# jklebes/MetropolisEngine

Measured on AMD Instinct MI355X. Metric: MC steps/sec (chains x sweeps) at 2^20 chains, 16 params, higher is better.
Workload: dtype f64

## Files before the change

### metropolisengine_amd/csrc/me_api.hip

```cpp
#include <algorithm>
#include <cmath>
#include <cstdlib>
#include <cstring>
#include <dlfcn.h>
#include <mutex>
#include <string>
#include <atomic>
#include <chrono>
#include <vector>

#include "me_comm.h"
#include "me_internal.h"

namespace me {

static std::vector<const KernelSet *> &registry() {
  static std::vector<const KernelSet *> sets;
  return sets;
}
static std::mutex &registry_mutex() {
  static std::mutex m;
  return m;
}
void register_kernel_set(const KernelSet *set) {
// ... 42 lines not shown
static bool host_factor(std::vector<double> &m, int nr, int nc) {
  auto tri = [](int i, int j) { return i * (i + 1) / 2 + j; };
  const int pr = nr * (nr + 1) / 2;
  auto cre = [pr](int i, int j) { return pr + i * i + 2 * j; };
  auto cim = [pr](int i, int j) { return pr + i * i + 2 * j + 1; };
  auto cdg = [pr](int i) { return pr + i * i + 2 * i; };
  for (int j = 0; j < nr; ++j) {
    double s = m[tri(j, j)];
    for (int k = 0; k < j; ++k) s -= m[tri(j, k)] * m[tri(j, k)];
    if (!(s > 0)) return false;
    const double dg = std::sqrt(s);
    m[tri(j, j)] = dg;
    for (int i = j + 1; i < nr; ++i) {
      double t = m[tri(i, j)];
      for (int k = 0; k < j; ++k) t -= m[tri(i, k)] * m[tri(j, k)];
      m[tri(i, j)] = t / dg;
    }
  }
  for (int j = 0; j < nc; ++j) {
    double s = m[cdg(j)];
    for (int k = 0; k < j; ++k) s -= m[cre(j, k)] * m[cre(j, k)] + m[cim(j, k)] * m[cim(j, k)];
    if (!(s > 0)) return false;
    const double dg = std::sqrt(s);
    m[cdg(j)] = dg;
    for (int i = j + 1; i < nc; ++i) {
      double tr = m[cre(i, j)], ti = m[cim(i, j)];
      for (int k = 0; k < j; ++k) {
        const double ar = m[cre(i, k)], ai = m[cim(i, k)], br = m[cre(j, k)], bi = m[cim(j, k)];
        tr -= ar * br + ai * bi;
        ti -= ai * br - ar * bi;
      }
      m[cre(i, j)] = tr / dg;
      m[cim(i, j)] = ti / dg;
    }
  }
  return true;
}

static bool initial_shape_is_identity(const me_config *c) {
  if (c->covariance_real)
    for (int i = 0; i < c->n_real; ++i)
      for (int j = 0; j <= i; ++j)
        if (c->covariance_real[i * c->n_real + j] != (i == j ? 1.0 : 0.0)) return false;
  if (c->covariance_complex)
    for (int i = 0; i < c->n_complex; ++i)
      for (int j = 0; j <= i; ++j) {
        const double re = c->covariance_complex[2 * (i * c->n_complex + j)], im = c->covariance_complex[2 * (i * c->n_complex + j) + 1];
        if (re != (i == j ? 1.0 : 0.0) || (i != j && im != 0.0)) return false;
      }
  return true;
}

}

using namespace me;

struct me_engine {
  int device = 0;
  hipStream_t stream = nullptr;
  bool own_stream = false;
  const KernelSet *ks = nullptr;
  int dtype = ME_F32;
  size_t esize = 4;
  long long n = 0;
  int nr = 0, nc = 0, d = 0, p = 0, nobs = 0;
  unsigned long long chain_offset = 0, seed = 0;
  double temp = 0, target_acceptance = 0.3, alpha = 0, ratio = 0, reject_bound = 0;
  int m = 0, energy_kind = 0, reject_kind = 0, cov_mode = 0;
  bool stale_total = false;
  hipEvent_t time_start = nullptr, time_stop = nullptr;
  std::vector<double> shared_host;
  int cov_kind = CK_IDENTITY;
  int grid_blocks = 0;
  int n_terms = 1;
  std::vector<double> coef;
  unsigned long long step_index = 0, measure_count = 1;
  unsigned long long fused_cycles = 0;
  void *x = nullptr, *energy = nullptr, *width = nullptr, *mean = nullptr, *cov = nullptr, *obs_mean = nullptr;
  void *factor = nullptr, *shared_factor = nullptr, *shared_full = nullptr, *shared_image = nullptr, *energy_image = nullptr, *coef_dev = nullptr,
       *row_dev = nullptr;
  unsigned long long *accept_slots = nullptr, *accept_total = nullptr;
  long long n_slots = 0;
  unsigned long long proposed = 0;
  bool x_tiled = false;
  int width_rows = 1;
  bool widths_synced = true;
  unsigned int *status = nullptr;
  double *pool_dev = nullptr, *pool_partials = nullptr, *pool_host = nullptr;
  unsigned long long *host_scratch = nullptr;
  hipStream_t copy_stream = nullptr;
  hipEvent_t pool_reduced = nullptr, pool_copied = nullptr;
  bool pool_pending = false;
  const RcclApi *rccl = nullptr;
  ncclComm_t comm = nullptr;
  int comm_rank = 0, comm_world = 1;
  double *trace_dev = nullptr;
  long long trace_chains = 0, trace_stride = 1, trace_rows = 0, trace_capacity = 0;
  std::string err;
};

namespace {

int fail(me_engine *e, int code, const std::string &msg) {
  if (e) e->err = msg;
  else g_create_error = msg;
  return code;
}

#define ME_HIP(e, call)                                                                                      \
  do {                                                                                                       \
    hipError_t err__ = (call);                                                                               \
    if (err__ != hipSuccess)                                                                                 \
      return fail((e), ME_ERR_HIP, std::string(#call) + ": " + hipGetErrorString(err__));                    \
  } while (0)

void to_device_type(const double *src, size_t count, int dtype, std::vector<unsigned char> &out) {
  out.resize(count * (dtype == ME_F32 ? 4 : 8));
  if (dtype == ME_F32) {
    float *o = reinterpret_cast<float *>(out.data());
    for (size_t i = 0; i < count; ++i) o[i] = (float)src[i];
  } else {
    std::memcpy(out.data(), src, count * 8);
  }
}

int broadcast(me_engine *e, void *dst, const std::vector<double> &row, bool tiled = false) {
  std::vector<unsigned char> bytes;
  to_device_type(row.data(), row.size(), e->dtype, bytes);
  ME_HIP(e, hipMemcpyAsync(e->row_dev, bytes.data(), bytes.size(), hipMemcpyHostToDevice, e->stream));
  if (tiled) ME_HIP(e, launch_broadcast_tiled(dst, e->row_dev, (int)row.size(), e->n, e->dtype, e->stream));
  else ME_HIP(e, launch_broadcast_rows(dst, e->row_dev, (int)row.size(), e->n, e->dtype, e->stream));
  ME_HIP(e, hipStreamSynchronize(e->stream));
  return ME_OK;
}

int check_status(me_engine *e);
int copy_tiled(me_engine *e, void *field_ptr, int entries, int64_t chain_begin, int64_t n_chains, double *dst, const double *src) {
  const int64_t tile0 = chain_begin >> 6, tile1 = (chain_begin + n_chains - 1) >> 6;
  const size_t tile_values = (size_t)entries * 64, n_values = (size_t)(tile1 - tile0 + 1) * tile_values;
  unsigned char *dev = (unsigned char *)field_ptr + (size_t)tile0 * tile_values * e->esize;
  std::vector<unsigned char> tmp(n_values * e->esize);
  const bool whole = (chain_begin & 63) == 0 && (((chain_begin + n_chains) & 63) == 0 || chain_begin + n_chains == e->n);
  if (dst || !whole) {
    ME_HIP(e, hipMemcpyAsync(tmp.data(), dev, tmp.size(), hipMemcpyDeviceToHost, e->stream));
    ME_HIP(e, hipStreamSynchronize(e->stream));
  }
  auto at = [&](int64_t c, int k) { return (size_t)((c >> 6) - tile0) * tile_values + (size_t)k * 64 + (size_t)(c & 63); };
  if (e->dtype == ME_F32) {
    float *t = reinterpret_cast<float *>(tmp.data());
    for (int64_t i = 0; i < n_chains; ++i)
      for (int k = 0; k < entries; ++k) {
        if (dst) dst[i * entries + k] = (double)t[at(chain_begin + i, k)];
        else t[at(chain_begin + i, k)] = (float)src[i * entries + k];
      }
  } else {
    double *t = reinterpret_cast<double *>(tmp.data());
    for (int64_t i = 0; i < n_chains; ++i)
      for (int k = 0; k < entries; ++k) {
        if (dst) dst[i * entries + k] = t[at(chain_begin + i, k)];
        else t[at(chain_begin + i, k)] = src[i * entries + k];
      }
  }
  if (src) {
    ME_HIP(e, hipMemcpyAsync(dev, tmp.data(), tmp.size(), hipMemcpyHostToDevice, e->stream));
    ME_HIP(e, hipStreamSynchronize(e->stream));
  }
  return dst ? check_status(e) : ME_OK;
}

int field_info(me_engine *e, int field, void **ptr, int *comps) {
  switch (field) {
    case ME_FIELD_PARAMS: *ptr = e->x; *comps = e->d; return ME_OK;
    case ME_FIELD_ENERGY: *ptr = e->energy; *comps = e->n_terms; return ME_OK;
    case ME_FIELD_WIDTH: *ptr = e->width; *comps = e->width_rows; return ME_OK;
    case ME_FIELD_MEAN: *ptr = e->mean; *comps = e->d; return ME_OK;
    case ME_FIELD_OBS_MEAN: *ptr = e->obs_mean; *comps = e->nobs; return ME_OK;
    case ME_FIELD_COV:
      if (!e->cov)
        return fail(e, ME_ERR_UNSUPPORTED, "this engine keeps no per-chain covariance: for large parameter spaces it is "
                                           "kept on request only (me_config.flags: ME_FLAG_TRACK_COVARIANCE), and not "
                                           "at all where the field would pass 4 GiB");
      *ptr = e->cov; *comps = e->p; return ME_OK;
    case ME_FIELD_ENERGY_TOTAL:
      if (!e->stale_total)
        return fail(e, ME_ERR_UNSUPPORTED, "this engine keeps one coherent energy ledger (sum ME_FIELD_ENERGY); a separate "
                                           "energy_total exists with ME_FLAG_REFERENCE_ENERGY_LEDGERS only");
      *ptr = (unsigned char *)e->energy + (size_t)e->n_terms * (size_t)e->n * e->esize; *comps = 1; return ME_OK;
    case ME_FIELD_FACTOR:
      if (!e->factor) return fail(e, ME_ERR_UNSUPPORTED, "this engine keeps no per-chain proposal factors (dimensions "
                                                         "without per-chain kernels, or a field beyond 4 GiB)");
      *ptr = e->factor; *comps = e->p; return ME_OK;
    default: return fail(e, ME_ERR_INVALID, "unknown field id");
  }
}

int report_status(me_engine *e, unsigned int bits) {
  if (!bits) return ME_OK;
  ME_HIP(e, hipMemsetAsync(e->status, 0, sizeof(unsigned int), e->stream));
  std::string msg = "numeric failure in at least one chain:";
  if (bits & ST_NONFINITE_ENERGY) msg += " non-finite energy;";
  if (bits & ST_BAD_PIVOT) msg += " non-positive Cholesky pivot (proposal covariance not positive definite);";
  if (bits & ST_BAD_WIDTH) msg += " sampling width <= 0;";
  return fail(e, ME_ERR_NUMERIC, msg);
}
int check_status(me_engine *e) {
  ME_HIP(e, hipMemcpyAsync(&e->host_scratch[0], e->status, sizeof(unsigned int), hipMemcpyDeviceToHost, e->stream));
  ME_HIP(e, hipStreamSynchronize(e->stream));
  return report_status(e, (unsigned int)e->host_scratch[0]);
}

int upload_shared_factor(me_engine *e, const double *packed) {
  std::vector<unsigned char> bytes;
  to_device_type(packed, (size_t)e->p, e->dtype, bytes);
  ME_HIP(e, hipMemcpy(e->shared_factor, bytes.data(), bytes.size(), hipMemcpyHostToDevice));
  if (e->shared_full) {
    std::vector<double> full((size_t)e->nr * e->nr, 0.0);
    for (int i = 0; i < e->nr; ++i)
      for (int j = 0; j <= i; ++j) full[(size_t)i * e->nr + j] = packed[i * (i + 1) / 2 + j];
    to_device_type(full.data(), full.size(), e->dtype, bytes);
    ME_HIP(e, hipMemcpy(e->shared_full, bytes.data(), bytes.size(), hipMemcpyHostToDevice));
    if (e->shared_image) ME_HIP(e, e->ks->prepare_matrix(e->shared_full, e->shared_image, e->stream));
  }
  return ME_OK;
}

void fill_step_launch(me_engine *e, StepLaunch &l, int n_sweeps) {
  l.n_real = e->nr;
  l.n_complex = e->nc;
  l.x = e->x;
  l.energy = e->energy;
// ... 129 lines not shown
      const bool dense = c->energy_kind == ME_ENERGY_DENSE_QUAD, pooled = c->cov_mode == ME_COV_POOLED || starts_shared;
      const bool per_chain = c->cov_mode == ME_COV_REFERENCE || (c->flags & ME_FLAG_TRACK_COVARIANCE) != 0;
      if ((dense || pooled || per_chain) && per_block * (pooled ? 2 : 1) > 150 * 1024)
        return fail(nullptr, ME_ERR_UNSUPPORTED,
                    "a dense quadratic form, a shared proposal factor or per-chain shapes beyond " + std::to_string(kMaxRegisterDof) +
                        " degrees of freedom are staged in LDS: this many parameters do not fit (float64: about 290, 145 with "
                        "a shared factor or an initial covariance that ME_COV_FIXED keeps; float32 twice that)");
    }
    if (c->flags & ME_FLAG_REFERENCE_ENERGY_LEDGERS)
      return fail(nullptr, ME_ERR_UNSUPPORTED, "ME_FLAG_REFERENCE_ENERGY_LEDGERS is not available beyond " +
                                                   std::to_string(kMaxRegisterDof) + " real degrees of freedom");
    if (c->reject_kind == ME_REJECT_USER) return fail(nullptr, ME_ERR_UNSUPPORTED, "no user plugins at these dimensions");
  }
  if ((c->flags & ME_FLAG_REFERENCE_ENERGY_LEDGERS) && (c->n_real == 0 || c->n_complex == 0))
    return fail(nullptr, ME_ERR_INVALID,
                "ME_FLAG_REFERENCE_ENERGY_LEDGERS applies to mixed engines (real and complex parameters): only their "
                "step_all keeps a separate energy_total (metropolis_engine.py:241-259)");
  if (c->cov_mode == ME_COV_REFERENCE && !ks->per_chain_cov)
    return fail(nullptr, ME_ERR_UNSUPPORTED,
                "per-chain adaptive covariance is not compiled for these dimensions; use ME_COV_FIXED or ME_COV_POOLED");

  bool keep_per_chain = ks->per_chain_cov && (!ks->streams_packed || c->cov_mode == ME_COV_REFERENCE);
  {
    const long long esz = c->dtype == ME_F32 ? 4 : 8;
    const long long limit = 1ll << 32;
    if (keep_per_chain && !ks->streams_packed && (long long)packed_total(c->n_real, c->n_complex) * ((c->n_chains + 63) / 64 * 64) * esz >= limit) {
      if (c->cov_mode == ME_COV_REFERENCE)
        return fail(nullptr, ME_ERR_UNSUPPORTED,
                    "the per-chain covariance field would exceed 4 GiB on this engine; shard the chains over more "
                    "engines or use ME_COV_FIXED / ME_COV_POOLED");
      keep_per_chain = false;
    }
    const long long rows = std::max<long long>(c->n_real + 2 * c->n_complex, 2 * c->n_real + c->n_complex);
    if (rows * ((c->n_chains + 63) / 64 * 64) * esz >= limit)
      return fail(nullptr, ME_ERR_UNSUPPORTED,
                  "a per-chain field would exceed 4 GiB on this engine; shard the chains over more engines");
  }
  int n_dev = 0;
  if (hipGetDeviceCount(&n_dev) != hipSuccess || n_dev <= 0)
    return fail(nullptr, ME_ERR_HIP, "no HIP device available (this library has no CPU fallback)");
  if (c->device_id < 0 || c->device_id >= n_dev) return fail(nullptr, ME_ERR_INVALID, "device_id out of range");

  me_engine *e = new me_engine;
  e->device = c->device_id;
  e->ks = ks;
  e->n_terms = ks->energy_terms(c->energy_kind);
  e->dtype = c->dtype;
  e->esize = c->dtype == ME_F32 ? 4 : 8;
  e->n = c->n_chains;
  e->nr = c->n_real;
  e->nc = c->n_complex;
  e->d = e->nr + 2 * e->nc;
  e->p = packed_total(e->nr, e->nc);
  e->nobs = n_observables(e->nr, e->nc);
  e->chain_offset = c->chain_offset;
  e->seed = c->seed;
  e->temp = c->temp;
  e->target_acceptance = c->target_acceptance;
  e->energy_kind = c->energy_kind;
  e->reject_kind = c->reject_kind;
  e->reject_bound = c->reject_bound;
  e->cov_mode = c->cov_mode;
  e->coef.assign(c->energy_coeffs, c->energy_coeffs + c->n_energy_coeffs);
  e->alpha = -norm_ppf(c->target_acceptance / 2.0);
  e->m = e->nr + e->nc;
  e->ratio = (1.0 - 1.0 / e->m) * std::sqrt(2.0 * M_PI) * std::exp(e->alpha * e->alpha / 2.0) / 2.0 * e->alpha +
             1.0 / (e->m * c->target_acceptance * (1.0 - c->target_acceptance));
  if (const char *g = std::getenv("ME_GRID_BLOCKS")) e->grid_blocks = std::atoi(g);

#define ME_CREATE_HIP(call)                                                                  \
  do {                                                                                       \
    hipError_t err__ = (call);                                                               \
    if (err__ != hipSuccess) {                                                               \
      g_create_error = std::string(#call) + ": " + hipGetErrorString(err__);                 \
      release(e);                                                                            \
      return ME_ERR_HIP;                                                                     \
    }                                                                                        \
  } while (0)

  ME_CREATE_HIP(hipSetDevice(e->device));
  ME_CREATE_HIP(hipStreamCreateWithFlags(&e->stream, hipStreamNonBlocking));
  e->own_stream = true;
  const size_t n = (size_t)e->n, es = e->esize;
  e->x_tiled = ks->tiled_state;
  ME_CREATE_HIP(hipMalloc(&e->x, (e->x_tiled ? (n + 63) / 64 * 64 : n) * e->d * es));
  e->stale_total = (c->flags & ME_FLAG_REFERENCE_ENERGY_LEDGERS) != 0;
  ME_CREATE_HIP(hipMalloc(&e->energy, n * (e->n_terms + (e->stale_total ? 1 : 0)) * es));
  e->width_rows = (e->nr > 0 && e->nc > 0) ? 3 : 1;
  ME_CREATE_HIP(hipMalloc(&e->width, n * e->width_rows * es));
  ME_CREATE_HIP(hipMalloc(&e->mean, n * e->d * es));
  ME_CREATE_HIP(hipMalloc(&e->obs_mean, n * e->nobs * es));
  if (keep_per_chain || ((!ks->per_chain_cov || ks->streams_packed) && ks->tracks_cov && (c->flags & ME_FLAG_TRACK_COVARIANCE)))
    ME_CREATE_HIP(hipMalloc(&e->cov, (n + 63) / 64 * 64 * e->p * es));
  if (keep_per_chain) ME_CREATE_HIP(hipMalloc(&e->factor, (n + 63) / 64 * 64 * e->p * es));
  ME_CREATE_HIP(hipMalloc(&e->shared_factor, (size_t)e->p * es));
  if (e->nc == 0) ME_CREATE_HIP(hipMalloc(&e->shared_full, (size_t)e->nr * e->nr * es));
  if (e->shared_full && ks->prepare_matrix) ME_CREATE_HIP(hipMalloc(&e->shared_image, ks->matrix_image_bytes));
  ME_CREATE_HIP(hipMalloc(&e->row_dev, (size_t)std::max(std::max(e->d, e->p), e->nobs) * es));
  e->n_slots = (e->n + 31) / 32 + 8;
  ME_CREATE_HIP(hipMalloc((void **)&e->accept_slots, (size_t)e->n_slots * sizeof(unsigned long long)));
  ME_CREATE_HIP(hipMalloc((void **)&e->accept_total, sizeof(unsigned long long)));
  ME_CREATE_HIP(hipMalloc((void **)&e->status, sizeof(unsigned int)));
  ME_CREATE_HIP(hipMalloc((void **)&e->pool_dev, sizeof(double) * (size_t)moments_size(e->nr, e->nc)));
  ME_CREATE_HIP(hipHostMalloc((void **)&e->host_scratch, 64, hipHostMallocDefault));
  e->host_scratch[0] = e->host_scratch[1] = 0;
  ME_CREATE_HIP(hipHostMalloc((void **)&e->pool_host, sizeof(double) * (size_t)moments_size(e->nr, e->nc), hipHostMallocDefault));
  if (pool_reduce_supported(e->nr, e->nc, e->dtype))
    ME_CREATE_HIP(hipMalloc((void **)&e->pool_partials,
                            sizeof(double) * (size_t)pool_reduce_blocks(e->n, e->nr, e->nc) *
                                (size_t)(1 + e->d + e->nr + e->nc + e->d * (e->d + 1) / 2)));
  ME_CREATE_HIP(hipMemsetAsync(e->accept_slots, 0, (size_t)e->n_slots * sizeof(unsigned long long), e->stream));
  ME_CREATE_HIP(hipMemsetAsync(e->status, 0, sizeof(unsigned int), e->stream));
  if (ks->n_real < 0 && e->energy_kind == ME_ENERGY_DIAG_QUAD) {
    if ((int)e->coef.size() != e->nr + e->nc) {
      g_create_error = "wrong number of energy coefficients for this energy kind";
      release(e);
      return ME_ERR_INVALID;
    }
    std::vector<double> expanded(e->coef.begin(), e->coef.begin() + e->nr);
    expanded.insert(expanded.end(), e->coef.begin() + e->nr, e->coef.end());
    expanded.insert(expanded.end(), e->coef.begin() + e->nr, e->coef.end());
    std::vector<unsigned char> bytes;
    to_device_type(expanded.data(), expanded.size(), e->dtype, bytes);
    ME_CREATE_HIP(hipMalloc(&e->coef_dev, bytes.size()));
    ME_CREATE_HIP(hipMemcpy(e->coef_dev, bytes.data(), bytes.size(), hipMemcpyHostToDevice));
  }
  if (ks->n_real < 0 && e->energy_kind == ME_ENERGY_DENSE_QUAD) {
    if ((int)e->coef.size() != e->d * e->d) {
      g_create_error = "wrong number of energy coefficients for this energy kind";
      release(e);
      return ME_ERR_INVALID;
    }
    std::vector<double> folded;
    folded.reserve((size_t)e->d * (e->d + 1) / 2);
    for (int i = 0; i < e->d; ++i)
      for (int j = 0; j <= i; ++j)
        folded.push_back(i == j ? e->coef[(size_t)i * e->d + i] : e->coef[(size_t)i * e->d + j] + e->coef[(size_t)j * e->d + i]);
    std::vector<unsigned char> bytes;
    to_device_type(folded.data(), folded.size(), e->dtype, bytes);
    ME_CREATE_HIP(hipMalloc(&e->coef_dev, bytes.size()));
    ME_CREATE_HIP(hipMemcpy(e->coef_dev, bytes.data(), bytes.size(), hipMemcpyHostToDevice));
  } else
  if (e->energy_kind == ME_ENERGY_DENSE_QUAD || (is_user_kind(e->energy_kind) && !e->coef.empty())) {
    std::vector<unsigned char> bytes;
    to_device_type(e->coef.data(), e->coef.size(), e->dtype, bytes);
    ME_CREATE_HIP(hipMalloc(&e->coef_dev, bytes.size()));
    ME_CREATE_HIP(hipMemcpy(e->coef_dev, bytes.data(), bytes.size(), hipMemcpyHostToDevice));
    if (e->energy_kind == ME_ENERGY_DENSE_QUAD && ks->prepare_matrix) {
      ME_CREATE_HIP(hipMalloc(&e->energy_image, ks->matrix_image_bytes));
      ME_CREATE_HIP(ks->prepare_matrix(e->coef_dev, e->energy_image, e->stream));
    }
  }
#undef ME_CREATE_HIP

  std::vector<double> init(c->initial_params, c->initial_params + e->d);
  std::vector<double> obs(e->nobs);
  for (int i = 0; i < e->nr; ++i) {
    obs[i] = std::fabs(init[i]);
    obs[e->nr + e->nc + i] = init[i] * init[i];
  }
  for (int j = 0; j < e->nc; ++j) obs[e->nr + j] = std::hypot(init[e->nr + j], init[e->nr + e->nc + j]);
  const int pr = packed_real(e->nr);
  std::vector<double> c0(e->p, 0.0);
  bool identity = true;
  for (int i = 0; i < e->nr; ++i)
    for (int j = 0; j <= i; ++j) {
      const double v = c->covariance_real ? c->covariance_real[i * e->nr + j] : (i == j ? 1.0 : 0.0);
      c0[i * (i + 1) / 2 + j] = v;
      identity = identity && v == (i == j ? 1.0 : 0.0);
    }
  for (int i = 0; i < e->nc; ++i) {
    for (int j = 0; j < i; ++j) {
      const double re = c->covariance_complex ? c->covariance_complex[2 * (i * e->nc + j)] : 0.0;
      const double im = c->covariance_complex ? c->covariance_complex[2 * (i * e->nc + j) + 1] : 0.0;
      c0[pr + i * i + 2 * j] = re;
      c0[pr + i * i + 2 * j + 1] = im;
      identity = identity && re == 0.0 && im == 0.0;
    }
    const double dg = c->covariance_complex ? c->covariance_complex[2 * (i * e->nc + i)] : 1.0;
    c0[pr + i * i + 2 * i] = dg;
    identity = identity && dg == 1.0;
  }
  std::vector<double> f0 = c0;
  for (int i = 0; i < e->nc; ++i)
    for (int j = 0; j < i; ++j) f0[pr + i * i + 2 * j + 1] = -f0[pr + i * i + 2 * j + 1];
  if (!host_factor(f0, e->nr, e->nc)) {
    release(e);
    return fail(nullptr, ME_ERR_INVALID, "initial covariance matrix is not positive definite (metropolis_engine.py:270)");
  }
  int rc = ME_OK;
  std::vector<double> width_row((size_t)e->width_rows, c->sampling_width);
  if ((rc = broadcast(e, e->x, init, e->x_tiled)) || (rc = broadcast(e, e->mean, init)) || (rc = broadcast(e, e->obs_mean, obs)) ||
      (rc = broadcast(e, e->width, width_row)) || (e->cov && (rc = broadcast(e, e->cov, c0, true))) ||
      (e->factor && (rc = broadcast(e, e->factor, f0, true)))) {
    g_create_error = e->err;
    release(e);
    return rc;
  }
  if (upload_shared_factor(e, f0.data()) != ME_OK) {
    g_create_error = e->err;
    release(e);
    return ME_ERR_HIP;
  }
  e->cov_kind = identity ? CK_IDENTITY : (ks->n_real < 0 && e->factor) ? CK_PER_CHAIN : CK_SHARED;

  rc = me_recompute_energy(e);
  if (rc == ME_OK) {
    hipError_t herr = hipStreamSynchronize(e->stream);
    if (herr != hipSuccess) rc = fail(e, ME_ERR_HIP, std::string("initial energy evaluation: ") + hipGetErrorString(herr));
  }
  if (rc != ME_OK) {
    g_create_error = e->err;
    release(e);
    return rc;
  }
  *out = e;
  return ME_OK;
}

int me_set_reject_condition(me_engine *e, int32_t reject_kind, double reject_bound) {
  if (!e) return ME_ERR_INVALID;
  if (reject_kind < ME_REJECT_NONE || reject_kind > ME_REJECT_USER) return fail(e, ME_ERR_INVALID, "unknown reject_kind");
  if (reject_kind == ME_REJECT_USER && e->energy_kind != ME_ENERGY_USER && e->energy_kind != ME_ENERGY_USER_INDIRECT)
    return fail(e, ME_ERR_INVALID, "ME_REJECT_USER needs a user-energy plugin (it supplies me_user_reject)");
  if (reject_kind == ME_REJECT_USER && !e->ks->has_user_reject)
    return fail(e, ME_ERR_UNSUPPORTED,
                "ME_REJECT_USER: this user-energy plugin defines no me_user_reject (#define ME_USER_HAS_REJECT in its source)");
  if (reject_kind == ME_REJECT_ABS_REAL0_GE && e->nr == 0)
    return fail(e, ME_ERR_INVALID, "ME_REJECT_ABS_REAL0_GE needs a real parameter");
  e->reject_kind = reject_kind;
  e->reject_bound = reject_bound;
  return ME_OK;
}

int me_set_energy(me_engine *e, int32_t energy_kind, const double *coeffs, int32_t n_coeffs, const char *user_name) {
  if (!e) return ME_ERR_INVALID;
  if (n_coeffs < 0 || (n_coeffs > 0 && !coeffs)) return fail(e, ME_ERR_INVALID, "energy coefficients missing");
  if (e->ks->n_real < 0) return fail(e, ME_ERR_UNSUPPORTED, "me_set_energy: not available on the runtime-dimension kernel set");
  if (energy_kind == ME_ENERGY_DENSE_QUAD)
    return fail(e, ME_ERR_UNSUPPORTED, "me_set_energy: the dense quadratic form keeps device images of its matrix; create a new engine");
  const KernelSet *ks = find_kernel_set(e->dtype, e->nr, e->nc, energy_kind, user_name);
  if (!ks || ks->n_real < 0)
    return fail(e, ME_ERR_UNSUPPORTED, is_user_kind(energy_kind)
                    ? std::string("no user-energy plugin named '") + (user_name ? user_name : "") + "' is loaded for these dimensions"
                    : "energy kind " + std::to_string(energy_kind) + " is not compiled for these dimensions");
  if (ks->tiled_state != e->ks->tiled_state || ks->per_chain_cov != e->ks->per_chain_cov || ks->streams_packed != e->ks->streams_packed ||
      ks->tracks_cov != e->ks->tracks_cov)
    return fail(e, ME_ERR_UNSUPPORTED, "me_set_energy: the plugin was built with other per-chain covariance options than this engine's kernel set");
  if (e->reject_kind == ME_REJECT_USER && !ks->has_user_reject)
    return fail(e, ME_ERR_UNSUPPORTED, "me_set_energy: the engine's wall is the plugin's me_user_reject, which the new energy does not define");
  const int n_terms = ks->energy_terms(energy_kind);
  ME_HIP(e, hipSetDevice(e->device));
  ME_HIP(e, hipStreamSynchronize(e->stream));
  if (n_terms != e->n_terms) {
    void *ledger = nullptr;
    ME_HIP(e, hipMalloc(&ledger, (size_t)e->n * (size_t)(n_terms + (e->stale_total ? 1 : 0)) * e->esize));
    (void)hipFree(e->energy);
    e->energy = ledger;
    e->n_terms = n_terms;
    if (e->trace_chains > 0) {
      if (e->trace_dev) (void)hipFree(e->trace_dev);
      e->trace_dev = nullptr;
      e->trace_rows = e->trace_capacity = 0;
    }
  }
  e->coef.assign(coeffs, coeffs + n_coeffs);
  if (e->coef_dev) {
    (void)hipFree(e->coef_dev);
    e->coef_dev = nullptr;
  }
  if (is_user_kind(energy_kind) && !e->coef.empty()) {
    std::vector<unsigned char> bytes;
    to_device_type(e->coef.data(), e->coef.size(), e->dtype, bytes);
    ME_HIP(e, hipMalloc(&e->coef_dev, bytes.size()));
    ME_HIP(e, hipMemcpy(e->coef_dev, bytes.data(), bytes.size(), hipMemcpyHostToDevice));
  }
  e->ks = ks;
  e->energy_kind = energy_kind;
  const int rc = me_recompute_energy(e);
  if (rc != ME_OK) return rc;
  ME_HIP(e, hipStreamSynchronize(e->stream));
  return check_status(e);
}

int me_load_plugin(const char *path) {
  if (!path) return fail(nullptr, ME_ERR_INVALID, "null plugin path");
  void *handle = dlopen(path, RTLD_NOW | RTLD_GLOBAL);
  if (!handle) return fail(nullptr, ME_ERR_INVALID, std::string("dlopen failed: ") + dlerror());
  return ME_OK;
}

int me_destroy(me_engine *e) {
  if (!e) return ME_ERR_INVALID;
  (void)hipSetDevice(e->device);
  if (e->stream) (void)hipStreamSynchronize(e->stream);
  if (e->copy_stream) (void)hipStreamSynchronize(e->copy_stream);
  release(e);
  return ME_OK;
}

int me_recompute_energy(me_engine *e) {
  if (!e) return ME_ERR_INVALID;
  ME_HIP(e, hipSetDevice(e->device));
  EnergyLaunch l;
  l.n_real = e->nr;
  l.n_complex = e->nc;
  l.total_row = e->stale_total ? e->n_terms : -1;
  l.x = e->x;
  l.energy = e->energy;
  l.coef_device = e->coef_dev;
  l.coef_host = e->coef.data();
  l.n_coef = (int)e->coef.size();
  l.status = e->status;
  l.n = e->n;
  l.energy_kind = e->energy_kind;
  l.grid_blocks = e->grid_blocks;
  hipError_t err = e->ks->init_energy(l, e->stream);
  if (err == hipErrorInvalidValue) return fail(e, ME_ERR_INVALID, "wrong number of energy coefficients for this energy kind");
  ME_HIP(e, err);
  return ME_OK;
}

static int split_widths(me_engine *e) {
  if (e->width_rows != 3 || !e->widths_synced) return ME_OK;
  const size_t row = (size_t)e->n * e->esize;
  for (int r = 1; r <= 2; ++r)
    ME_HIP(e, hipMemcpyAsync((unsigned char *)e->width + r * row, e->width, row, hipMemcpyDeviceToDevice, e->stream));
  e->widths_synced = false;
  return ME_OK;
// ... 45 lines not shown

int me_step(me_engine *e, int32_t n_sweeps) { return me_step_kind(e, ME_STEP_ALL, n_sweeps); }

int me_step_kind(me_engine *e, int32_t kind, int32_t n_sweeps) {
  if (!e) return ME_ERR_INVALID;
  if (n_sweeps <= 0) return fail(e, ME_ERR_INVALID, "n_sweeps must be positive");
  ME_HIP(e, hipSetDevice(e->device));
  return launch_step_kind(e, kind, n_sweeps, nullptr, nullptr);
}

int me_step_injected(me_engine *e, int32_t kind, int32_t n_sweeps, const double *normals, const double *uniforms) {
  if (!e || !normals || !uniforms) return ME_ERR_INVALID;
  if (n_sweeps <= 0) return fail(e, ME_ERR_INVALID, "n_sweeps must be positive");
  if (e->dtype != ME_F64) return fail(e, ME_ERR_UNSUPPORTED, "injected-stream replay is compiled for float64 engines only");
  ME_HIP(e, hipSetDevice(e->device));
  const bool magphase = kind == ME_STEP_COMPLEX_MAGNITUDE_PHASE;
  const size_t n = (size_t)e->n, k = (size_t)n_sweeps;
  const size_t nz = magphase ? (size_t)e->nc : (size_t)e->d, nu = magphase ? (size_t)e->nc + 2 : 1;
  std::vector<double> zn(k * nz * n), un(k * nu * n);
  for (size_t s = 0; s < k; ++s)
    for (size_t c = 0; c < n; ++c) {
      for (size_t j = 0; j < nz; ++j) zn[(s * nz + j) * n + c] = normals[(s * n + c) * nz + j];
      for (size_t j = 0; j < nu; ++j) un[(s * nu + j) * n + c] = uniforms[(s * n + c) * nu + j];
    }
  double *zd = nullptr, *ud = nullptr;
  ME_HIP(e, hipMalloc((void **)&zd, zn.size() * sizeof(double)));
  hipError_t herr = hipMalloc((void **)&ud, un.size() * sizeof(double));
  if (herr != hipSuccess) {
    (void)hipFree(zd);
    return fail(e, ME_ERR_HIP, "hipMalloc of the injected uniforms failed");
  }
  int rc = ME_OK;
  if (hipMemcpy(zd, zn.data(), zn.size() * sizeof(double), hipMemcpyHostToDevice) != hipSuccess ||
      hipMemcpy(ud, un.data(), un.size() * sizeof(double), hipMemcpyHostToDevice) != hipSuccess) {
    rc = fail(e, ME_ERR_HIP, "upload of the injected streams failed");
  } else {
    rc = launch_step_kind(e, kind, n_sweeps, zd, ud);
    if (rc == ME_OK && hipStreamSynchronize(e->stream) != hipSuccess) rc = fail(e, ME_ERR_HIP, "injected step failed");
  }
  (void)hipFree(zd);
  (void)hipFree(ud);
  return rc;
}

namespace {
void fill_measure_launch(me_engine *e, MeasureLaunch &l, unsigned long long count) {
  l.n_real = e->nr;
  l.n_complex = e->nc;
  l.x = e->x;
  l.width = e->width;
  l.mean = e->mean;
  l.cov = e->cov;
  l.obs_mean = e->obs_mean;
  l.factor = e->factor;
  l.status = e->status;
  l.n = e->n;
  l.measure_count = count;
  l.update_cov = (count > 50 && e->cov) ? 1 : 0;
  l.split_widths = (e->width_rows == 3 && !e->widths_synced) ? 1 : 0;
  l.write_factor = (l.update_cov && e->cov_mode == ME_COV_REFERENCE) ? 1 : 0;
  l.grid_blocks = e->grid_blocks;
}

int commit_measure(me_engine *e, const MeasureLaunch &l) {
  e->measure_count = l.measure_count;
  if (l.write_factor) e->cov_kind = CK_PER_CHAIN;
  if (e->trace_chains > 0) {
    const long long cols = e->d + e->n_terms + e->width_rows;
    if (e->trace_rows == e->trace_capacity) {
      const long long cap = e->trace_capacity ? 2 * e->trace_capacity : 1024;
      double *bigger = nullptr;
      ME_HIP(e, hipMalloc((void **)&bigger, sizeof(double) * (size_t)(cap * cols * e->trace_chains)));
      if (e->trace_dev) {
        ME_HIP(e, hipMemcpyAsync(bigger, e->trace_dev, sizeof(double) * (size_t)(e->trace_rows * cols * e->trace_chains),
                                 hipMemcpyDeviceToDevice, e->stream));
        ME_HIP(e, hipStreamSynchronize(e->stream));
        (void)hipFree(e->trace_dev);
      }
      e->trace_dev = bigger;
      e->trace_capacity = cap;
    }
    const int rows_valid = (e->width_rows == 3 && e->widths_synced) ? 1 : e->width_rows;
    ME_HIP(e, launch_trace(e->x, e->energy, e->width, e->n, e->d, e->n_terms, rows_valid, e->dtype, e->trace_chains, e->trace_stride,
                           e->trace_dev + e->trace_rows * cols * e->trace_chains, e->stream, e->x_tiled));
    if (rows_valid != e->width_rows) {
      double *row = e->trace_dev + e->trace_rows * cols * e->trace_chains + (size_t)(e->d + e->n_terms) * e->trace_chains;
      for (int r = 1; r < 3; ++r)
        ME_HIP(e, hipMemcpyAsync(row + (size_t)r * e->trace_chains, row, sizeof(double) * (size_t)e->trace_chains,
                                 hipMemcpyDeviceToDevice, e->stream));
    }
    e->trace_rows += 1;
  }
  return ME_OK;
}
}

int me_measure(me_engine *e) {
  if (!e) return ME_ERR_INVALID;
  ME_HIP(e, hipSetDevice(e->device));
  MeasureLaunch l;
  fill_measure_launch(e, l, e->measure_count + 1);
  ME_HIP(e, e->ks->measure(l, e->stream));
  return commit_measure(e, l);
}

int me_cycle(me_engine *e, int32_t n_sweeps) {
  if (!e) return ME_ERR_INVALID;
  if (n_sweeps <= 0) return fail(e, ME_ERR_INVALID, "n_sweeps must be positive");
  ME_HIP(e, hipSetDevice(e->device));
  if (e->ks->cycle) {
    StepLaunch sl;
    fill_step_launch(e, sl, n_sweeps);
    MeasureLaunch ml;
    fill_measure_launch(e, ml, e->measure_count + 1);
    ml.split_widths = 0;
    const hipError_t err = e->ks->cycle(sl, ml, e->stream);
    if (err == hipSuccess) {
      e->widths_synced = true;
      e->step_index += (unsigned long long)n_sweeps;
      e->proposed += (unsigned long long)e->n * (unsigned long long)n_sweeps;
      e->fused_cycles += 1;
      return commit_measure(e, ml);
    }
    if (err != hipErrorNotSupported) ME_HIP(e, err);
    (void)hipGetLastError();
  }
  const int rc = me_step(e, n_sweeps);
  return rc != ME_OK ? rc : me_measure(e);
}

int me_cycle_stats(me_engine *e, uint64_t *fused_cycles) {
  if (!e || !fused_cycles) return ME_ERR_INVALID;
  *fused_cycles = e->fused_cycles;
  return ME_OK;
}

int me_trace_enable(me_engine *e, int64_t n_traced, int64_t stride) {
  if (!e) return ME_ERR_INVALID;
  if (n_traced < 0 || stride < 1 || (n_traced > 0 && (n_traced - 1) * stride >= e->n))
    return fail(e, ME_ERR_INVALID, "traced chains out of range");
  ME_HIP(e, hipSetDevice(e->device));
  ME_HIP(e, hipStreamSynchronize(e->stream));
  if (e->trace_dev) (void)hipFree(e->trace_dev);
  e->trace_dev = nullptr;
  e->trace_chains = n_traced;
  e->trace_stride = stride;
  e->trace_rows = e->trace_capacity = 0;
  return ME_OK;
}

int me_trace_shape(me_engine *e, int64_t *rows, int64_t *cols, int64_t *n_traced) {
  if (!e) return ME_ERR_INVALID;
  if (rows) *rows = e->trace_rows;
  if (cols) *cols = e->d + e->n_terms + e->width_rows;
  if (n_traced) *n_traced = e->trace_chains;
  return ME_OK;
}

int me_trace_get(me_engine *e, double *dst, int64_t n_doubles) {
  if (!e || !dst) return ME_ERR_INVALID;
  const long long want = e->trace_rows * (e->d + e->n_terms + e->width_rows) * e->trace_chains;
  if (n_doubles != want) return fail(e, ME_ERR_INVALID, "wrong trace buffer length");
  if (want == 0) return ME_OK;
  ME_HIP(e, hipSetDevice(e->device));
  ME_HIP(e, hipStreamSynchronize(e->stream));
  ME_HIP(e, hipMemcpy(dst, e->trace_dev, sizeof(double) * (size_t)want, hipMemcpyDeviceToHost));
  return ME_OK;
}

int me_field_components(me_engine *e, int32_t field, int32_t *n_components) {
  if (!e || !n_components) return ME_ERR_INVALID;
  void *ptr;
  int comps;
  int rc = field_info(e, field, &ptr, &comps);
  if (rc == ME_OK) *n_components = comps;
  return rc;
}

int me_energy_terms(me_engine *e, int32_t *n_terms) {
  if (!e || !n_terms) return ME_ERR_INVALID;
  *n_terms = e->n_terms;
  return ME_OK;
}

int me_get(me_engine *e, int32_t field, int64_t chain_begin, int64_t n_chains, double *dst) {
  if (!e || !dst) return ME_ERR_INVALID;
  if (chain_begin < 0 || n_chains < 0 || chain_begin + n_chains > e->n) return fail(e, ME_ERR_INVALID, "chain range out of bounds");
  ME_HIP(e, hipSetDevice(e->device));
  void *ptr;
  int comps;
  int rc = field_info(e, field, &ptr, &comps);
  if (rc != ME_OK) return rc;
  if (n_chains == 0) return ME_OK;
  if (field == ME_FIELD_COV || field == ME_FIELD_FACTOR || (field == ME_FIELD_PARAMS && e->x_tiled))
    return copy_tiled(e, ptr, comps, chain_begin, n_chains, dst, nullptr);
  std::vector<unsigned char> tmp((size_t)comps * n_chains * e->esize);
  for (int r = 0; r < comps; ++r)
    ME_HIP(e, hipMemcpyAsync(tmp.data() + (size_t)r * n_chains * e->esize,
                             (const unsigned char *)ptr + ((size_t)r * e->n + chain_begin) * e->esize,
                             (size_t)n_chains * e->esize, hipMemcpyDeviceToHost, e->stream));
  ME_HIP(e, hipStreamSynchronize(e->stream));
  if (e->dtype == ME_F32) {
    const float *t = reinterpret_cast<const float *>(tmp.data());
    for (int r = 0; r < comps; ++r)
      for (int64_t c = 0; c < n_chains; ++c) dst[c * comps + r] = (double)t[(size_t)r * n_chains + c];
  } else {
    const double *t = reinterpret_cast<const double *>(tmp.data());
    for (int r = 0; r < comps; ++r)
      for (int64_t c = 0; c < n_chains; ++c) dst[c * comps + r] = t[(size_t)r * n_chains + c];
  }
  if (field == ME_FIELD_WIDTH && e->width_rows == 3 && e->widths_synced)
    for (int64_t c = 0; c < n_chains; ++c) dst[c * 3 + 1] = dst[c * 3 + 2] = dst[c * 3];
  return check_status(e);
}

int me_set(me_engine *e, int32_t field, int64_t chain_begin, int64_t n_chains, const double *src) {
  if (!e || !src) return ME_ERR_INVALID;
  if (chain_begin < 0 || n_chains < 0 || chain_begin + n_chains > e->n) return fail(e, ME_ERR_INVALID, "chain range out of bounds");
  ME_HIP(e, hipSetDevice(e->device));
  void *ptr;
  int comps;
  int rc = field_info(e, field, &ptr, &comps);
  if (rc != ME_OK) return rc;
  if (field == ME_FIELD_WIDTH && e->width_rows == 3 && (chain_begin != 0 || n_chains != e->n))
    return fail(e, ME_ERR_INVALID, "widths of a mixed engine must be set for all chains at once");
  if (n_chains == 0) return ME_OK;
  if (field == ME_FIELD_COV || field == ME_FIELD_FACTOR || (field == ME_FIELD_PARAMS && e->x_tiled)) {
    rc = copy_tiled(e, ptr, comps, chain_begin, n_chains, nullptr, src);
    if (rc != ME_OK) return rc;
    if (field == ME_FIELD_FACTOR) e->cov_kind = CK_PER_CHAIN;
    return ME_OK;
  }
  std::vector<unsigned char> tmp((size_t)comps * n_chains * e->esize);
  if (e->dtype == ME_F32) {
    float *t = reinterpret_cast<float *>(tmp.data());
    for (int r = 0; r < comps; ++r)
      for (int64_t c = 0; c < n_chains; ++c) t[(size_t)r * n_chains + c] = (float)src[c * comps + r];
  } else {
    double *t = reinterpret_cast<double *>(tmp.data());
    for (int r = 0; r < comps; ++r)
      for (int64_t c = 0; c < n_chains; ++c) t[(size_t)r * n_chains + c] = src[c * comps + r];
  }
  for (int r = 0; r < comps; ++r)
    ME_HIP(e, hipMemcpyAsync((unsigned char *)ptr + ((size_t)r * e->n + chain_begin) * e->esize,
                             tmp.data() + (size_t)r * n_chains * e->esize, (size_t)n_chains * e->esize,
                             hipMemcpyHostToDevice, e->stream));
  ME_HIP(e, hipStreamSynchronize(e->stream));
  if (field == ME_FIELD_FACTOR) e->cov_kind = CK_PER_CHAIN;
  if (field == ME_FIELD_WIDTH && e->width_rows == 3) e->widths_synced = false;
  return ME_OK;
}

int me_constants(me_engine *e, double *alpha, int32_t *m, double *ratio) {
  if (!e) return ME_ERR_INVALID;
  if (alpha) *alpha = e->alpha;
  if (m) *m = e->m;
  if (ratio) *ratio = e->ratio;
  return ME_OK;
}

int me_counters(me_engine *e, uint64_t *step_index, uint64_t *measure_step_counter) {
  if (!e) return ME_ERR_INVALID;
  if (step_index) *step_index = e->step_index;
  if (measure_step_counter) *measure_step_counter = e->measure_count;
  return ME_OK;
}

int me_set_counters(me_engine *e, uint64_t step_index, uint64_t measure_step_counter) {
  if (!e) return ME_ERR_INVALID;
  if (measure_step_counter < 1) return fail(e, ME_ERR_INVALID, "measure_step_counter starts at 1");
  e->step_index = step_index;
  e->measure_count = measure_step_counter;
  return ME_OK;
}

int me_accept_stats(me_engine *e, uint64_t *accepted, uint64_t *proposed) {
  if (!e) return ME_ERR_INVALID;
  ME_HIP(e, hipSetDevice(e->device));
  ME_HIP(e, launch_sum_slots(e->accept_slots, e->n_slots, e->accept_total, e->stream));
  ME_HIP(e, hipMemcpyAsync(&e->host_scratch[1], e->accept_total, sizeof(unsigned long long), hipMemcpyDeviceToHost, e->stream));
  ME_HIP(e, hipMemcpyAsync(&e->host_scratch[0], e->status, sizeof(unsigned int), hipMemcpyDeviceToHost, e->stream));
  ME_HIP(e, hipStreamSynchronize(e->stream));
  if (accepted) *accepted = e->host_scratch[1];
  if (proposed) *proposed = e->proposed;
  return report_status(e, (unsigned int)e->host_scratch[0]);
}

int me_set_accept_stats(me_engine *e, uint64_t accepted, uint64_t proposed) {
  if (!e) return ME_ERR_INVALID;
  if (accepted > proposed) return fail(e, ME_ERR_INVALID, "accepted exceeds proposed");
  ME_HIP(e, hipSetDevice(e->device));
  const unsigned long long total = accepted;
  ME_HIP(e, hipMemsetAsync(e->accept_slots, 0, (size_t)e->n_slots * sizeof(unsigned long long), e->stream));
  ME_HIP(e, hipMemcpyAsync(e->accept_slots, &total, sizeof(total), hipMemcpyHostToDevice, e->stream));
  ME_HIP(e, hipStreamSynchronize(e->stream));
  e->proposed = proposed;
  return ME_OK;
}

int me_pooled_moments_size(me_engine *e, int64_t *n_doubles) {
  if (!e || !n_doubles) return ME_ERR_INVALID;
  *n_doubles = moments_size(e->nr, e->nc);
  return ME_OK;
}

namespace {
int enqueue_pooled_moments(me_engine *e, void *device_out, int64_t n_doubles) {
  if (n_doubles != moments_size(e->nr, e->nc)) return fail(e, ME_ERR_INVALID, "wrong pooled-moment buffer length");
  if (e->pool_pending) return fail(e, ME_ERR_STATE, "a pooled-moment reduction is in flight (me_pooled_moments_end first)");
  if (!e->pool_partials) return fail(e, ME_ERR_UNSUPPORTED, "pooled moments: dimension too large for the reduction kernel");
  ME_HIP(e, hipSetDevice(e->device));
  hipError_t err = launch_pool_reduce(e->x, e->n, e->nr, e->nc, e->dtype, e->accept_slots, e->n_slots,
                                      (double)e->proposed, e->pool_partials, (double *)device_out, e->stream,
                                      e->ks->pool_stage1, e->x_tiled);
  if (err == hipErrorInvalidValue) return fail(e, ME_ERR_UNSUPPORTED, "pooled moments: dimension too large for the reduction kernel");
  ME_HIP(e, err);
  return ME_OK;
}
}

static hipError_t wait_polling(hipEvent_t ev) {
  const auto t0 = std::chrono::steady_clock::now();
  for (;;) {
    const hipError_t rc = hipEventQuery(ev);
    if (rc != hipErrorNotReady) return rc;
    if (std::chrono::steady_clock::now() - t0 > std::chrono::milliseconds(2)) return hipEventSynchronize(ev);
  }
}
static hipError_t wait_polling(hipStream_t stream) {
  const auto t0 = std::chrono::steady_clock::now();
  for (;;) {
    const hipError_t rc = hipStreamQuery(stream);
    if (rc != hipErrorNotReady) return rc;
    if (std::chrono::steady_clock::now() - t0 > std::chrono::milliseconds(2)) return hipStreamSynchronize(stream);
  }
}

int me_pooled_moments_device(me_engine *e, void *device_out, int64_t n_doubles) {
  if (!e || !device_out) return ME_ERR_INVALID;
  int rc = enqueue_pooled_moments(e, device_out, n_doubles);
  if (rc != ME_OK) return rc;
  ME_HIP(e, wait_polling(e->stream));
  return ME_OK;
}

int me_pooled_moments(me_engine *e, double *host_out, int64_t n_doubles) {
  if (!e || !host_out) return ME_ERR_INVALID;
  int rc = enqueue_pooled_moments(e, e->pool_dev, n_doubles);
  if (rc != ME_OK) return rc;
  ME_HIP(e, hipMemcpyAsync(e->pool_host, e->pool_dev, sizeof(double) * (size_t)n_doubles, hipMemcpyDeviceToHost, e->stream));
  ME_HIP(e, wait_polling(e->stream));
  std::memcpy(host_out, e->pool_host, sizeof(double) * (size_t)n_doubles);
  return ME_OK;
}

namespace {
int begin_pooled(me_engine *e, bool allreduce) {
  if (e->pool_pending) return fail(e, ME_ERR_STATE, "a pooled-moment reduction is already in flight: call me_pooled_moments_end first");
  if (allreduce && !e->comm)
    return fail(e, ME_ERR_STATE, "this engine has no communicator: call me_comm_init_rank first (single-GPU engines use me_pooled_moments)");
  ME_HIP(e, hipSetDevice(e->device));
  if (!e->copy_stream) {
    ME_HIP(e, hipStreamCreateWithFlags(&e->copy_stream, hipStreamNonBlocking));
    ME_HIP(e, hipEventCreateWithFlags(&e->pool_reduced, hipEventDisableTiming));
    ME_HIP(e, hipEventCreateWithFlags(&e->pool_copied, hipEventDisableTiming));
  }
  const int64_t n_doubles = moments_size(e->nr, e->nc);
  int rc = enqueue_pooled_moments(e, e->pool_dev, n_doubles);
  if (rc != ME_OK) return rc;
  ME_HIP(e, hipEventRecord(e->pool_reduced, e->stream));
  ME_HIP(e, hipStreamWaitEvent(e->copy_stream, e->pool_reduced, 0));
  if (allreduce) {
    const ncclResult_t nrc = e->rccl->all_reduce(e->pool_dev, e->pool_dev, (size_t)n_doubles, ncclDouble, ncclSum, e->comm, e->copy_stream);
    if (nrc != ncclSuccess) return fail(e, ME_ERR_HIP, std::string("ncclAllReduce: ") + e->rccl->error_string(nrc));
  }
  ME_HIP(e, hipMemcpyAsync(e->pool_host, e->pool_dev, sizeof(double) * (size_t)n_doubles, hipMemcpyDeviceToHost, e->copy_stream));
  ME_HIP(e, hipEventRecord(e->pool_copied, e->copy_stream));
  e->pool_pending = true;
  return ME_OK;
}
}

int me_pooled_moments_begin(me_engine *e) {
  if (!e) return ME_ERR_INVALID;
  return begin_pooled(e, false);
}

int me_pooled_moments_allreduce_begin(me_engine *e) {
  if (!e) return ME_ERR_INVALID;
  return begin_pooled(e, true);
}

int me_pooled_moments_allreduce(me_engine *e, double *host_out, int64_t n_doubles) {
  if (!e || !host_out) return ME_ERR_INVALID;
  if (n_doubles != moments_size(e->nr, e->nc)) return fail(e, ME_ERR_INVALID, "wrong pooled-moment buffer length");
  const int rc = begin_pooled(e, true);
  return rc != ME_OK ? rc : me_pooled_moments_end(e, host_out, n_doubles);
// ... 193 lines not shown
```

### metropolisengine_amd/csrc/me_device.h

```cpp
#pragma once

#include <type_traits>
#include <utility>

#include <hip/hip_runtime.h>
#include <stdint.h>

#include "me_internal.h"
#include "me_math64.h"

namespace me {

struct U4 {
  uint32_t x, y, z, w;
};

__device__ __forceinline__ uint32_t xor3(uint32_t a, uint32_t b, uint32_t c) {
  return __builtin_amdgcn_bitop3_b32(a, b, c, 0x96);
}
__device__ __forceinline__ U4 philox4x32_10(U4 c, uint32_t k0, uint32_t k1) {
#pragma unroll
  for (int r = 0; r < 10; ++r) {
    const uint64_t p0 = (uint64_t)0xD2511F53u * c.x;
    const uint64_t p1 = (uint64_t)0xCD9E8D57u * c.z;
// ... 111 lines not shown
                                            (unsigned int)row * row_bytes, ME_NT_AUX);
    } else {
      using v2 = decltype(__builtin_amdgcn_raw_buffer_load_b64(rsrc, 0u, 0u, 0));
      __builtin_amdgcn_raw_buffer_store_b64(__builtin_bit_cast(v2, value), rsrc, chain_off,
                                            (unsigned int)row * row_bytes, ME_NT_AUX);
    }
  }
  __device__ __forceinline__ void store(int row, unsigned int chain_off, R value) const {
    if constexpr (sizeof(R) == 4) {
      __builtin_amdgcn_raw_buffer_store_b32(__builtin_bit_cast(unsigned int, value), rsrc, chain_off,
                                            (unsigned int)row * row_bytes, 0);
    } else {
      using v2 = decltype(__builtin_amdgcn_raw_buffer_load_b64(rsrc, 0u, 0u, 0));
      __builtin_amdgcn_raw_buffer_store_b64(__builtin_bit_cast(v2, value), rsrc, chain_off,
                                            (unsigned int)row * row_bytes, 0);
    }
  }
};

template <typename R>
__device__ __forceinline__ unsigned int tiled_offset(long long c, int entries) {
  return (unsigned int)(((c >> 6) * (long long)entries * 64 + (c & 63)) * (long long)sizeof(R));
}
template <typename R>
struct TiledField {
  __amdgpu_buffer_rsrc_t rsrc;
  __device__ __forceinline__ TiledField(const R *base, long long n, int entries)
      : rsrc(__builtin_amdgcn_make_buffer_rsrc(const_cast<R *>(base), 0,
                                               (unsigned int)(((n + 63) >> 6) * (long long)entries * 64 * (long long)sizeof(R)),
                                               0x00020000)) {}
  static constexpr unsigned int kEntryBytes = 64u * (unsigned int)sizeof(R);
  template <int AUX>
  __device__ __forceinline__ R load_aux(int k, unsigned int tile_off) const {
    if constexpr (sizeof(R) == 4) {
      return __builtin_bit_cast(R, __builtin_amdgcn_raw_buffer_load_b32(rsrc, tile_off, (unsigned int)k * kEntryBytes, AUX));
    } else {
      const auto v = __builtin_amdgcn_raw_buffer_load_b64(rsrc, tile_off, (unsigned int)k * kEntryBytes, AUX);
      return __builtin_bit_cast(R, v);
    }
  }
  template <int AUX>
  __device__ __forceinline__ void store_aux(int k, unsigned int tile_off, R value) const {
    if constexpr (sizeof(R) == 4) {
      __builtin_amdgcn_raw_buffer_store_b32(__builtin_bit_cast(unsigned int, value), rsrc, tile_off, (unsigned int)k * kEntryBytes, AUX);
    } else {
      using v2 = decltype(__builtin_amdgcn_raw_buffer_load_b64(rsrc, 0u, 0u, 0));
      __builtin_amdgcn_raw_buffer_store_b64(__builtin_bit_cast(v2, value), rsrc, tile_off, (unsigned int)k * kEntryBytes, AUX);
    }
  }
  __device__ __forceinline__ R load(int k, unsigned int tile_off) const { return load_aux<0>(k, tile_off); }
  __device__ __forceinline__ R load_nt(int k, unsigned int tile_off) const { return load_aux<ME_NT_AUX>(k, tile_off); }
  __device__ __forceinline__ void store(int k, unsigned int tile_off, R value) const { store_aux<0>(k, tile_off, value); }
  __device__ __forceinline__ void store_nt(int k, unsigned int tile_off, R value) const { store_aux<ME_NT_AUX>(k, tile_off, value); }
};

template <bool NT, class F>
__device__ __forceinline__ auto packed_load(const F &f, int row, unsigned int chain_off) {
  if constexpr (NT) return f.load_nt(row, chain_off);
  else return f.load(row, chain_off);
}
template <bool NT, class F, typename R>
__device__ __forceinline__ void packed_store(const F &f, int row, unsigned int chain_off, R value) {
  if constexpr (NT) f.store_nt(row, chain_off, value);
  else f.store(row, chain_off, value);
}

template <typename R, bool NTS>
struct StateField : Field<R> {
  using Field<R>::Field;
  __device__ __forceinline__ R load(int row, unsigned int chain_off) const {
    if constexpr (NTS) return Field<R>::load_nt(row, chain_off);
    else return Field<R>::load(row, chain_off);
  }
  __device__ __forceinline__ void store(int row, unsigned int chain_off, R value) const {
    if constexpr (NTS) Field<R>::store_nt(row, chain_off, value);
    else Field<R>::store(row, chain_off, value);
  }
};

#ifndef ME_TILED_STATE_DOF
#define ME_TILED_STATE_DOF 16
#endif
constexpr int kTiledStateDof = ME_TILED_STATE_DOF;
template <typename R, int D, bool NTS = false>
struct XField {
  static constexpr bool kTiled = D >= kTiledStateDof;
  std::conditional_t<kTiled, TiledField<R>, StateField<R, NTS>> f;
  __device__ __forceinline__ XField(const R *base, long long n) : f(base, n, D) {}
  static __device__ __forceinline__ unsigned int offset(long long c) {
    if constexpr (kTiled) return tiled_offset<R>(c, D);
    else return (unsigned int)c * (unsigned int)sizeof(R);
  }
  __device__ __forceinline__ R load(int row, unsigned int off) const {
    if constexpr (kTiled && NTS) return f.load_nt(row, off);
    else return f.load(row, off);
  }
  __device__ __forceinline__ void store(int row, unsigned int off, R value) const {
    if constexpr (kTiled && NTS) f.store_nt(row, off, value);
    else f.store(row, off, value);
  }
};
template <typename R, int D>
__device__ __forceinline__ long long state_index(long long c, int row, long long n) {
  if constexpr (D >= kTiledStateDof) return ((c >> 6) * (long long)D + row) * 64 + (c & 63);
  else return (long long)row * n + c;
}

constexpr int kMaxPackedInRegisters = 160;
#ifndef ME_STREAM_F64_ENTRIES
#define ME_STREAM_F64_ENTRIES 96
#endif
constexpr int kStreamF64Entries = ME_STREAM_F64_ENTRIES;

template <typename R, int NR, int NC>
struct EnergyIso {
  static constexpr int D = NR + 2 * NC;
  R a;
  __device__ __forceinline__ R operator()(const R (&x)[D]) const {
    R s0 = 0, s1 = 0;
#pragma unroll
    for (int d = 0; d + 1 < D; d += 2) {
      s0 += x[d] * x[d];
      s1 += x[d + 1] * x[d + 1];
    }
    if constexpr (D % 2 == 1) s0 += x[D - 1] * x[D - 1];
    return a * (s0 + s1);
  }
};

template <typename R, int NR, int NC>
struct EnergyDiag {
  static constexpr int D = NR + 2 * NC;
  R w[D];
  __device__ __forceinline__ R operator()(const R (&x)[D]) const {
    R s0 = 0, s1 = 0;
#pragma unroll
    for (int d = 0; d + 1 < D; d += 2) {
      s0 += w[d] * x[d] * x[d];
      s1 += w[d + 1] * x[d + 1] * x[d + 1];
    }
    if constexpr (D % 2 == 1) s0 += w[D - 1] * x[D - 1] * x[D - 1];
    return s0 + s1;
  }
};

template <typename R, int NR, int NC>
struct EnergyDense {
  static constexpr int D = NR + 2 * NC;
  static constexpr int PT = D * (D + 1) / 2;
  const R *a;
  static __device__ __forceinline__ R *folded() {
    __shared__ R t[PT];
    return t;
  }
  __device__ __forceinline__ void prepare() const {
    R *t = folded();
    constexpr int kBatch = 8;
    for (int k0 = threadIdx.x; k0 < PT; k0 += kBatch * (int)blockDim.x) {
      R lo[kBatch], hi[kBatch];
#pragma unroll
      for (int u = 0; u < kBatch; ++u) {
        const int k = k0 + u * (int)blockDim.x;
        lo[u] = hi[u] = R(0);
        if (k < PT) {
          int i = (int)((__builtin_sqrtf((float)(8 * k + 1)) - 1.0f) * 0.5f);
          if ((i + 1) * (i + 2) / 2 <= k) ++i;
          if (i * (i + 1) / 2 > k) --i;
          const int j = k - i * (i + 1) / 2;
          lo[u] = a[i * D + j];
          if (i != j) hi[u] = a[j * D + i];
        }
      }
#pragma unroll
      for (int u = 0; u < kBatch; ++u) {
        const int k = k0 + u * (int)blockDim.x;
        if (k < PT) t[k] = lo[u] + hi[u];
      }
    }
    __syncthreads();
  }
  __device__ __forceinline__ R operator()(const R (&x)[D]) const {
    const R *t = folded();
    asm volatile("" ::: "memory");
    R e = 0;
#pragma unroll
    for (int i = 0; i < D; ++i) {
      R y = 0;
#pragma unroll
// ... 185 lines not shown
#pragma unroll
    for (int j = 0; j < D; ++j) g[j] = a.inj_normals[((long long)s * D + j) * a.n + c];
    u = a.inj_uniforms[(long long)s * a.n + c];
  } else {
    uint32_t words[4 * NBLK];
#pragma unroll
    for (int b = 0; b < NBLK; ++b) {
      U4 ctr;
      ctr.x = (uint32_t)gid;
      ctr.y = (uint32_t)(gid >> 32);
      ctr.z = (uint32_t)step;
      ctr.w = ((uint32_t)(step >> 32) << 16) | (uint32_t)b;
      const U4 o = philox4x32_10(ctr, a.seed_lo, a.seed_hi);
      words[4 * b + 0] = o.x;
      words[4 * b + 1] = o.y;
      words[4 * b + 2] = o.z;
      words[4 * b + 3] = o.w;
    }
#pragma unroll
    for (int q = 0; q < NW / 2; ++q) N_::normal_pair(words[2 * q], words[2 * q + 1], g[2 * q], g[2 * q + 1]);
    u = N_::unit(words[NW]);
  }

}

template <typename R, int NR, int NC, int CK, int GROUP, class Fac>
__device__ __forceinline__ void propose_registers(const R (&x)[NR + 2 * NC], const R (&g)[2 * ((NR + 2 * NC + 1) / 2)], R w_r, R w_c,
                                                  Fac &&fac, R (&xp)[NR + 2 * NC]) {
  constexpr int D = NR + 2 * NC;
  [[maybe_unused]] constexpr int PR = NR * (NR + 1) / 2;
  constexpr bool MOVE_REAL = NR > 0 && GROUP != GROUP_COMPLEX;
  constexpr bool MOVE_COMPLEX = NC > 0 && GROUP != GROUP_REAL;
#pragma unroll
  for (int d = 0; d < D; ++d) xp[d] = x[d];
  if constexpr (CK == CK_IDENTITY) {
    if constexpr (MOVE_REAL) {
#pragma unroll
      for (int i = 0; i < NR; ++i) xp[i] = x[i] + w_r * g[i];
    }
    if constexpr (MOVE_COMPLEX) {
#pragma unroll
      for (int j = 0; j < NC; ++j) {
        xp[NR + j] = x[NR + j] + w_c * (g[NR + j] * R(0.70710678118654752440));
        xp[NR + NC + j] = x[NR + NC + j] + w_c * (g[NR + NC + j] * R(0.70710678118654752440));
      }
    }
  } else {
    if constexpr (MOVE_REAL) {
#pragma unroll
      for (int i = 0; i < NR; ++i) {
        R acc = 0;
#pragma unroll
        for (int j = 0; j <= i; ++j) acc += fac(tri(i, j)) * g[j];
        xp[i] = x[i] + w_r * acc;
      }
    }
    if constexpr (MOVE_COMPLEX) {
#pragma unroll
      for (int i = 0; i < NC; ++i) {
        R are = 0, aim = 0;
#pragma unroll
        for (int j = 0; j < i; ++j) {
          const R lre = fac(cre(PR, i, j));
          const R lim = fac(cim(PR, i, j));
          const R wre = g[NR + j] * R(0.70710678118654752440), wim = g[NR + NC + j] * R(0.70710678118654752440);
          are += lre * wre - lim * wim;
          aim += lre * wim + lim * wre;
        }
        const R ld = fac(cdiag(PR, i));
        are += ld * (g[NR + i] * R(0.70710678118654752440));
        aim += ld * (g[NR + NC + i] * R(0.70710678118654752440));
        xp[NR + i] = x[NR + i] + w_c * are;
        xp[NR + NC + i] = x[NR + NC + i] + w_c * aim;
      }
    }
  }

}

template <typename R, int NR, int NC, class Energy, int CK, int GROUP, class Ledger>
__device__ __forceinline__ void decide_step(const StepArgs<R> &a, const Energy &en, bool stale_total, R u,
                                            const R (&g)[2 * ((NR + 2 * NC + 1) / 2)], R (&x)[NR + 2 * NC], const R (&xp)[NR + 2 * NC],
                                            Ledger &ledger, R &total_q5, R &w, R &w_r, R &w_c, unsigned int &wave_accepted,
                                            bool &bad_energy) {
  [[maybe_unused]] constexpr int D = NR + 2 * NC;
  constexpr bool MOVE_REAL = NR > 0 && GROUP != GROUP_COMPLEX;
  constexpr bool MOVE_COMPLEX = NC > 0 && GROUP != GROUP_REAL;
  using N_ = Num<R>;
  bool rejected = false;
  if (a.reject_kind == ME_REJECT_ABS_REAL0_GE) rejected = !(N_::abs_(xp[0]) < a.reject_bound);
  else if (a.reject_kind == ME_REJECT_USER) rejected = energy_reject(en, xp, 0);
  R terms_new[Ledger::T];
  const R e_new = ledger.propose(en, xp, terms_new);
  const R diff = e_new - (stale_total ? total_q5 : ledger.partial());
  bool accept = diff <= R(0);
  if (a.temp > R(0)) accept = accept || N_::uphill(u, diff, a.inv_temp, a.inv_temp_log2e);
  accept = accept && !rejected;
  bad_energy |= (!rejected && !N_::finite(e_new));
  if constexpr (CK == CK_IDENTITY) {
    const R wa_r = accept ? w_r : R(0), wa_c = accept ? w_c : R(0);
    if constexpr (MOVE_REAL) {
#pragma unroll
      for (int i = 0; i < NR; ++i) x[i] = x[i] + wa_r * g[i];
    }
    if constexpr (MOVE_COMPLEX) {
#pragma unroll
      for (int j = 0; j < NC; ++j) {
        x[NR + j] = x[NR + j] + wa_c * (g[NR + j] * R(0.70710678118654752440));
        x[NR + NC + j] = x[NR + NC + j] + wa_c * (g[NR + NC + j] * R(0.70710678118654752440));
      }
    }
  } else {
#pragma unroll
    for (int d = 0; d < D; ++d) x[d] = accept ? xp[d] : x[d];
  }
  if (stale_total) total_q5 = accept ? e_new : total_q5;
  else ledger.commit(accept, terms_new);
  w = N_::adapt(w, accept, a.ratio, a.p, a.damping, a.up, a.down);
  if constexpr (GROUP == GROUP_ALL) w_r = w_c = w;
  else if constexpr (GROUP == GROUP_REAL) w_r = w;
  else w_c = w;
  wave_accepted += (unsigned int)__popcll(__ballot(accept));
}

template <typename R, int NR, int NC, class Energy, int CK, bool INJECT, int GROUP, class Ledger, class Fac>
__device__ __forceinline__ void run_sweeps(const StepArgs<R> &a, const Energy &en, long long c, unsigned long long gid,
                                           bool stale_total, R (&x)[NR + 2 * NC], Ledger &ledger, R &total_q5, R &w, R &w_r,
                                           R &w_c, Fac &&fac, unsigned int &wave_accepted, bool &bad_energy) {
  constexpr int D = NR + 2 * NC;
  constexpr int NW = 2 * ((D + 1) / 2);
  for (int s = 0; s < a.n_sweeps; ++s) {
    R g[NW], u, xp[D];
    draw_step<R, NR, NC, INJECT>(a, c, gid, s, g, u);
    propose_registers<R, NR, NC, CK, GROUP>(x, g, w_r, w_c, fac, xp);
    decide_step<R, NR, NC, Energy, CK, GROUP>(a, en, stale_total, u, g, x, xp, ledger, total_q5, w, w_r, w_c, wave_accepted, bad_energy);
  }
}

#ifndef ME_STEP_WAVES_PER_EU
#define ME_STEP_WAVES_PER_EU 0
#endif
#if ME_STEP_WAVES_PER_EU > 0
#define ME_STEP_BOUNDS __launch_bounds__(kFusedStepThreads, ME_STEP_WAVES_PER_EU)
#else
#define ME_STEP_BOUNDS __launch_bounds__(kFusedStepThreads)
#endif

#ifndef ME_STEP_PRIO_SHIFT
#define ME_STEP_PRIO_SHIFT 8
#endif
__device__ __forceinline__ void stagger_priority() {
#if ME_STEP_PRIO_SHIFT >= 0
  switch ((blockIdx.x >> ME_STEP_PRIO_SHIFT) & 3u) {
    case 0: __builtin_amdgcn_s_setprio(3); break;
    case 1: __builtin_amdgcn_s_setprio(2); break;
    case 2: __builtin_amdgcn_s_setprio(1); break;
    default: break;
  }
#endif
}

template <typename R, int NR, int NC, class Energy, int CK, bool INJECT = false, int GROUP = GROUP_ALL, bool NTS = false>
__global__ void ME_STEP_BOUNDS k_step(StepArgs<R> a, Energy en) {
  constexpr int D = NR + 2 * NC;
  constexpr bool MIXED = NR > 0 && NC > 0;
  static_assert(GROUP == GROUP_ALL || MIXED, "group-wise kernels exist for mixed engines only");
  using N_ = Num<R>;

  stagger_priority();
  if constexpr (!INJECT) N_::prepare();
  energy_prepare(en, 0);
  unsigned int wave_accepted = 0;
  bool bad_energy = false, bad_width = false;
  const long long stride = (long long)gridDim.x * blockDim.x;
  using Ledger = EnergyLedger<R, Energy, GROUP>;
  const XField<R, D, NTS> fx(a.x, a.n);
  const StateField<R, NTS> fe(a.energy, a.n, Ledger::T + (MIXED ? 1 : 0)), fw(a.width, a.n, MIXED ? 3 : 1);
  const bool stale_total = MIXED && GROUP == GROUP_ALL && a.stale_total != 0;
  constexpr bool PER_CHAIN = CK == CK_PER_CHAIN || CK == CK_PER_CHAIN_NT;
  constexpr int PF = PER_CHAIN ? NR * (NR + 1) / 2 + NC * NC : 0;
  constexpr bool STREAM_FACTOR = PER_CHAIN && (PF > kMaxPackedInRegisters ||
                                               (!INJECT && sizeof(R) == 8 && NC == 0 && PF > kStreamF64Entries));
  const TiledField<R> ffac(a.factor, a.n, STREAM_FACTOR ? 0 : PF);
  for (long long c = (long long)blockIdx.x * blockDim.x + threadIdx.x; c < a.n; c += stride) {
    const unsigned int coff = (unsigned int)c * (unsigned int)sizeof(R);
    const unsigned int xoff = fx.offset(c);
    R x[D];
#pragma unroll
    for (int d = 0; d < D; ++d) x[d] = fx.load(d, xoff);
    Ledger ledger;
    R total_q5 = R(0);
    if (stale_total) total_q5 = fe.load(Ledger::T, coff);
    else ledger.load(fe, coff);
    R w = fw.load(MIXED ? GROUP : 0, coff);
    R w_r = w, w_c = w;
    if constexpr (MIXED && GROUP == GROUP_ALL) {
      if (a.split_widths) {
        w_r = fw.load(GROUP_REAL, coff);
        w_c = fw.load(GROUP_COMPLEX, coff);
      }
    }
    const unsigned long long gid = a.chain_offset + (unsigned long long)c;
    [[maybe_unused]] const unsigned int toff = tiled_offset<R>(c, PF);
    auto fac = [&](int k) -> R {
      if constexpr (CK == CK_PER_CHAIN_NT) return ffac.load_nt(k, toff);
      else if constexpr (CK == CK_PER_CHAIN) return ffac.load(k, toff);
      else return a.factor[k];
    };

    if constexpr (STREAM_FACTOR) {
      constexpr int NW = 2 * ((D + 1) / 2);
      for (int s = 0; s < a.n_sweeps; ++s) {
        static_assert(!INJECT, "the streamed-factor form has no replay hook");
        constexpr int NBLK = (NW + 1 + 3) / 4;
        const unsigned long long step = a.step_index + (unsigned long long)s;
        R g[NW];
        R u_accept;
        {
          uint32_t words[4 * NBLK];
#pragma unroll
          for (int b = 0; b < NBLK; ++b) {
            U4 ctr;
            ctr.x = (uint32_t)gid;
            ctr.y = (uint32_t)(gid >> 32);
            ctr.z = (uint32_t)step;
            ctr.w = ((uint32_t)(step >> 32) << 16) | (uint32_t)b;
            const U4 o = philox4x32_10(ctr, a.seed_lo, a.seed_hi);
            words[4 * b + 0] = o.x;
            words[4 * b + 1] = o.y;
            words[4 * b + 2] = o.z;
            words[4 * b + 3] = o.w;
          }
#pragma unroll
          for (int q = 0; q < NW / 2; ++q) N_::normal_pair(words[2 * q], words[2 * q + 1], g[2 * q], g[2 * q + 1]);
          u_accept = N_::unit(words[NW]);
        }
        R xp[D];
#pragma unroll
        for (int d = 0; d < D; ++d) xp[d] = x[d];
        asm volatile("" ::: "memory");
        constexpr int CH = (int)(ME_STREAM_CHUNK_BYTES / sizeof(R));
        const R *tile_base = a.factor + (c >> 6) * (long long)PF * 64;
        const unsigned long long tb = (unsigned long long)tile_base;
        const R *tile_uniform = (const R *)join_halves(__builtin_amdgcn_readfirstlane((int)(tb >> 32)),
                                                       __builtin_amdgcn_readfirstlane((int)(unsigned int)tb));
        const __amdgpu_buffer_rsrc_t tile = __builtin_amdgcn_make_buffer_rsrc(const_cast<R *>(tile_uniform), 0,
                                                                               (unsigned int)(PF * 64 * sizeof(R)), 0x00020000);
        const unsigned int lane_off = (unsigned int)(c & 63) * (unsigned int)sizeof(R);
        auto entry = [&](int k) -> R {
          constexpr int AUX = CK == CK_PER_CHAIN_NT ? ME_NT_AUX : 0;
          if constexpr (sizeof(R) == 4)
            return __builtin_bit_cast(R, __builtin_amdgcn_raw_buffer_load_b32(tile, lane_off, (unsigned int)k * 64u * 4u, AUX));
          else
            return __builtin_bit_cast(R, __builtin_amdgcn_raw_buffer_load_b64(tile, lane_off, (unsigned int)k * 64u * 8u, AUX));
        };
        R f[2][CH];
#pragma unroll
        for (int u = 0; u < CH; ++u)
          if (u < PF) f[0][u] = entry(u);
        auto use = [&](auto entry_index) -> R {
          constexpr int k = decltype(entry_index)::value;
          if constexpr (k % CH == 0) {
            __builtin_amdgcn_sched_barrier(0);
#pragma unroll
            for (int u = 0; u < CH; ++u)
              if (k + CH + u < PF) f[(k / CH + 1) & 1][u] = entry(k + CH + u);
            __builtin_amdgcn_sched_barrier(0);
          }
          return f[(k / CH) & 1][k % CH];
        };
        static_for<NR>([&](auto row_index) {
          constexpr int i = decltype(row_index)::value;
          R acc = 0;
          static_for<i + 1>([&](auto col_index) {
            constexpr int j = decltype(col_index)::value, k = tri(i, j);
            const R l = use(std::integral_constant<int, k>{});
            acc = j == 0 ? l * g[0] : acc + l * g[j];
          });
          if constexpr (GROUP != GROUP_COMPLEX) xp[i] = x[i] + w_r * acc;
        });
        static_for<NC>([&](auto row_index) {
          constexpr int i = decltype(row_index)::value;
          R are = 0, aim = 0;
          static_for<i>([&](auto col_index) {
            constexpr int j = decltype(col_index)::value;
            const R lre = use(std::integral_constant<int, cre(NR * (NR + 1) / 2, i, j)>{});
            const R lim = use(std::integral_constant<int, cim(NR * (NR + 1) / 2, i, j)>{});
            const R wre = g[NR + j] * R(0.70710678118654752440), wim = g[NR + NC + j] * R(0.70710678118654752440);
            are += lre * wre - lim * wim;
            aim += lre * wim + lim * wre;
          });
          const R ld = use(std::integral_constant<int, cdiag(NR * (NR + 1) / 2, i)>{});
          are += ld * (g[NR + i] * R(0.70710678118654752440));
          aim += ld * (g[NR + NC + i] * R(0.70710678118654752440));
          if constexpr (GROUP != GROUP_REAL) {
            xp[NR + i] = x[NR + i] + w_c * are;
            xp[NR + NC + i] = x[NR + NC + i] + w_c * aim;
          }
        });
        bool rejected = false;
        if (a.reject_kind == ME_REJECT_ABS_REAL0_GE) rejected = !(N_::abs_(xp[0]) < a.reject_bound);
        else if (a.reject_kind == ME_REJECT_USER) rejected = energy_reject(en, xp, 0);
        R terms_new[Ledger::T];
        const R e_new = ledger.propose(en, xp, terms_new);
        const R diff = e_new - (stale_total ? total_q5 : ledger.partial());
        bool accept = diff <= R(0);
        if (a.temp > R(0)) accept = accept || N_::uphill(u_accept, diff, a.inv_temp, a.inv_temp_log2e);
        accept = accept && !rejected;
        bad_energy |= (!rejected && !N_::finite(e_new));
#pragma unroll
        for (int d = 0; d < D; ++d) x[d] = accept ? xp[d] : x[d];
        if (stale_total) total_q5 = accept ? e_new : total_q5;
        else ledger.commit(accept, terms_new);
        w = N_::adapt(w, accept, a.ratio, a.p, a.damping, a.up, a.down);
        if constexpr (GROUP == GROUP_ALL) w_r = w_c = w;
        else if constexpr (GROUP == GROUP_REAL) w_r = w;
        else w_c = w;
        wave_accepted += (unsigned int)__popcll(__ballot(accept));
      }
    } else {
      run_sweeps<R, NR, NC, Energy, CK, INJECT, GROUP>(a, en, c, gid, stale_total, x, ledger, total_q5, w, w_r, w_c, fac, wave_accepted, bad_energy);
    }
    bad_width |= !(w > R(0));
#pragma unroll
    for (int d = 0; d < D; ++d) fx.store(d, xoff, x[d]);
    if (stale_total) fe.store(Ledger::T, coff, total_q5);
    else ledger.store(fe, coff);
    fw.store(MIXED ? GROUP : 0, coff, w);
  }
  if ((threadIdx.x & 63) == 0 && wave_accepted) {
    unsigned long long *slot = a.accept_slots + (size_t)blockIdx.x * (blockDim.x >> 6) + (threadIdx.x >> 6);
    *slot += (unsigned long long)wave_accepted;
  }
  const unsigned int bits = (bad_energy ? ST_NONFINITE_ENERGY : 0u) | (bad_width ? ST_BAD_WIDTH : 0u);
  if (bits) atomicOr(a.status, bits);
}

template <typename R, int NR, int NC, class Energy>
__global__ void __launch_bounds__(kStepThreads) k_init_energy(const R *xs, R *energy, long long n, unsigned int *status,
                                                                Energy en, int total_row) {
  constexpr int D = NR + 2 * NC;
  energy_prepare(en, 0);
  const long long stride = (long long)gridDim.x * kStepThreads;
  for (long long c = (long long)blockIdx.x * kStepThreads + threadIdx.x; c < n; c += stride) {
    R x[D];
#pragma unroll
    for (int d = 0; d < D; ++d) x[d] = xs[state_index<R, D>(c, d, n)];
    constexpr int T = term_count<Energy>::value;
    bool finite = true;
    R total = R(0);
#pragma unroll
    for (int t = 0; t < T; ++t) {
      R e;
      if constexpr (T == 1) e = en(x);
      else e = en.term(t, x);
      energy[(long long)t * n + c] = e;
      total = t == 0 ? e : total + e;
      finite = finite && Num<R>::finite(e);
    }
    if (total_row >= 0) energy[(long long)total_row * n + c] = total;
    if (!finite) atomicOr(status, (unsigned int)ST_NONFINITE_ENERGY);
  }
}

template <typename R>
struct MeasureArgs {
  const R *x, *width;
  R *mean, *cov, *obs_mean, *factor;
  unsigned int *status;
  long long n;
  R keep;
  R inv_i;
  R cov_keep;
  int update_cov, write_factor, split_widths;
};

template <typename R, int NR, int NC>
__device__ __forceinline__ void cholesky_packed(R (&m)[NR * (NR + 1) / 2 + NC * NC], bool &bad_pivot) {
  constexpr int PR = NR * (NR + 1) / 2;
  using N_ = Num<R>;
#pragma unroll
    for (int j = 0; j < NR; ++j) {
      R s = m[tri(j, j)];
#pragma unroll
      for (int k = 0; k < j; ++k) s = fma_(-m[tri(j, k)], m[tri(j, k)], s);
      if (!(s > R(0))) { bad_pivot = true; s = R(1e-30); }
      const R dg = N_::sqrt_(s);
      const R inv = R(1) / dg;
      m[tri(j, j)] = dg;
#pragma unroll
      for (int i = j + 1; i < NR; ++i) {
        R t = m[tri(i, j)];
#pragma unroll
        for (int k = 0; k < j; ++k) t = fma_(-m[tri(i, k)], m[tri(j, k)], t);
        m[tri(i, j)] = t * inv;
      }
    }
#pragma unroll
    for (int j = 0; j < NC; ++j) {
      R s = m[cdiag(PR, j)];
#pragma unroll
      for (int k = 0; k < j; ++k) s = fma_(-m[cim(PR, j, k)], m[cim(PR, j, k)], fma_(-m[cre(PR, j, k)], m[cre(PR, j, k)], s));
      if (!(s > R(0))) { bad_pivot = true; s = R(1e-30); }
      const R dg = N_::sqrt_(s);
      const R inv = R(1) / dg;
      m[cdiag(PR, j)] = dg;
#pragma unroll
      for (int i = j + 1; i < NC; ++i) {
// ... 121 lines not shown
            R v[16];
#pragma unroll
            for (int u = 0; u < 16; ++u) v[u] = p[u * ts];
#pragma unroll
            for (int u = 0; u < 8; ++u) {
              const R aj = s_delta[NR + j + u][threadIdx.x], bj = s_delta[NR + NC + j + u][threadIdx.x];
              p[(2 * u) * ts] = fma_(fma_(ai, aj, bi * bj), a.inv_i, v[2 * u] * a.cov_keep);
              p[(2 * u + 1) * ts] = fma_(fma_(bi, aj, -(ai * bj)), a.inv_i, v[2 * u + 1] * a.cov_keep);
            }
            p += 16 * ts;
          }
          for (; j < i; ++j) {
            const R aj = s_delta[NR + j][threadIdx.x], bj = s_delta[NR + NC + j][threadIdx.x];
            const R re = p[0], im = p[ts];
            p[0] = fma_(fma_(ai, aj, bi * bj), a.inv_i, re * a.cov_keep);
            p[ts] = fma_(fma_(bi, aj, -(ai * bj)), a.inv_i, im * a.cov_keep);
            p += 2 * ts;
          }
          *p = fma_(w2_cplx, a.inv_i, fma_(fma_(ai, ai, bi * bi), a.inv_i, *p * a.cov_keep));
          p += ts;
        }
      } else {
      R m[P];
#pragma unroll
      for (int k = 0; k < P; ++k) m[k] = src.cov(k);
#pragma unroll
      for (int i = 0; i < NR; ++i)
#pragma unroll
        for (int j = 0; j <= i; ++j) {
          const int k = tri(i, j);
          R v = fma_(delta[i] * delta[j], a.inv_i, m[k] * a.cov_keep);
          if (i == j) v = fma_(w2_real, a.inv_i, v);
          packed_store<NT>(fcov, k, toff, v);
          m[k] = v;
        }
#pragma unroll
      for (int i = 0; i < NC; ++i) {
        const R ai = delta[NR + i], bi = delta[NR + NC + i];
#pragma unroll
        for (int j = 0; j < i; ++j) {
          const R aj = delta[NR + j], bj = delta[NR + NC + j];
          const int kr = cre(PR, i, j), ki = cim(PR, i, j);
          const R vr = fma_(fma_(ai, aj, bi * bj), a.inv_i, m[kr] * a.cov_keep);
          const R vi = fma_(fma_(bi, aj, -(ai * bj)), a.inv_i, m[ki] * a.cov_keep);
          packed_store<NT>(fcov, kr, toff, vr);
          packed_store<NT>(fcov, ki, toff, vi);
          m[kr] = vr;
          m[ki] = -vi;
        }
        const int kd = cdiag(PR, i);
        const R vd = fma_(w2_cplx, a.inv_i, fma_(fma_(ai, ai, bi * bi), a.inv_i, m[kd] * a.cov_keep));
        packed_store<NT>(fcov, kd, toff, vd);
        m[kd] = vd;
      }
      if constexpr (FUSED) {
        if (a.write_factor) {
          cholesky_packed<R, NR, NC>(m, bad_pivot);
#pragma unroll
          for (int k = 0; k < P; ++k) packed_store<NT>(ffac, k, toff, m[k]);
        }
      }
      }
    }
  }
}

template <typename R, int NR, int NC, bool PER_CHAIN_COV, bool FUSED, bool NT, bool NTM>
__global__ void __launch_bounds__(kStepThreads, ME_MEASURE_WAVES) k_measure(MeasureArgs<R> a) {
  constexpr int D = NR + 2 * NC;
  constexpr int P = NR * (NR + 1) / 2 + NC * NC;
  constexpr int NOBS = 2 * NR + NC;
  bool bad_pivot = false;
  const long long stride = (long long)gridDim.x * kStepThreads;
  const XField<R, D> fx(a.x, a.n);
  const Field<R> fw(a.width, a.n, (NR > 0 && NC > 0) ? 3 : 1), fmean(a.mean, a.n, D), fobs(a.obs_mean, a.n, NOBS);
  constexpr bool STREAM = PER_CHAIN_COV && P > kMaxPackedInRegisters;
  const TiledField<R> fcov(a.cov, a.n, (PER_CHAIN_COV && !STREAM) ? P : 0);
  const TiledField<R> ffac(a.factor, a.n, (PER_CHAIN_COV && FUSED) ? P : 0);
  __shared__ R s_delta[STREAM ? D : 1][kStepThreads];
  for (long long c = (long long)blockIdx.x * kStepThreads + threadIdx.x; c < a.n; c += stride) {
    const unsigned int coff = (unsigned int)c * (unsigned int)sizeof(R);
    const unsigned int xoff = fx.offset(c);
    R x[D];
#pragma unroll
    for (int d = 0; d < D; ++d) x[d] = fx.load(d, xoff);
    const MeasureFromMemory<R, NT, NTM> src{fmean, fobs, fcov, coff, tiled_offset<R>(c, P)};
    measure_chain<R, NR, NC, PER_CHAIN_COV, FUSED, NT, NTM>(a, c, x, src, fmean, fobs, fcov, ffac, s_delta, [&](R &w_real, R &w_cplx) {
      constexpr bool MIXED = NR > 0 && NC > 0;
      w_real = fw.load((MIXED && a.split_widths) ? 1 : 0, coff);
      w_cplx = fw.load((MIXED && a.split_widths) ? 2 : 0, coff);
    }, bad_pivot);
  }
  if (bad_pivot) atomicOr(a.status, (unsigned int)ST_BAD_PIVOT);
}

#ifndef ME_CYCLE_PREFETCH
#define ME_CYCLE_PREFETCH 0
#endif
constexpr int cycle_prefetch_level(int, int, int, int) { return ME_CYCLE_PREFETCH; }

template <typename R, int NR, int NC, class Energy, int CK, bool NT, bool NTM>
__global__ void ME_STEP_BOUNDS k_cycle(StepArgs<R> a, MeasureArgs<R> ma, Energy en) {
  constexpr int D = NR + 2 * NC;
  constexpr int P = NR * (NR + 1) / 2 + NC * NC;
  constexpr int NOBS = 2 * NR + NC;
  constexpr bool MIXED = NR > 0 && NC > 0;
  static_assert(P <= kMaxPackedInRegisters, "k_cycle keeps the packed matrix in registers");
  static_assert(CK == CK_IDENTITY || CK == CK_SHARED || CK == CK_PER_CHAIN, "NT selects the non-temporal factor read");
  constexpr int CKX = CK == CK_PER_CHAIN ? (NT ? CK_PER_CHAIN_NT : CK_PER_CHAIN) : CK;
  using N_ = Num<R>;
  N_::prepare();
  energy_prepare(en, 0);
  unsigned int wave_accepted = 0;
  bool bad_energy = false, bad_width = false, bad_pivot = false;
  const long long stride = (long long)gridDim.x * blockDim.x;
  using Ledger = EnergyLedger<R, Energy, GROUP_ALL>;
  const XField<R, D> fx(a.x, a.n);
  const Field<R> fe(a.energy, a.n, Ledger::T + (MIXED ? 1 : 0)), fw(a.width, a.n, MIXED ? 3 : 1);
  const Field<R> fmean(ma.mean, a.n, D), fobs(ma.obs_mean, a.n, NOBS);
  const TiledField<R> fcov(ma.cov, a.n, P), ffac(ma.factor, a.n, P);
  const bool stale_total = MIXED && a.stale_total != 0;
  for (long long c = (long long)blockIdx.x * blockDim.x + threadIdx.x; c < a.n; c += stride) {
    const unsigned int coff = (unsigned int)c * (unsigned int)sizeof(R);
    const unsigned int xoff = fx.offset(c);
    R x[D];
#pragma unroll
    for (int d = 0; d < D; ++d) x[d] = fx.load(d, xoff);
    Ledger ledger;
    R total_q5 = R(0);
    if (stale_total) total_q5 = fe.load(Ledger::T, coff);
    else ledger.load(fe, coff);
    R w = fw.load(0, coff);
    R w_r = w, w_c = w;
    if constexpr (MIXED) {
      if (a.split_widths) {
        w_r = fw.load(GROUP_REAL, coff);
        w_c = fw.load(GROUP_COMPLEX, coff);
      }
    }
    const unsigned long long gid = a.chain_offset + (unsigned long long)c;
    [[maybe_unused]] const unsigned int toff = tiled_offset<R>(c, P);
    auto fac = [&](int k) -> R {
      if constexpr (CK == CK_PER_CHAIN) return packed_load<NT>(ffac, k, toff);
      else return a.factor[k];
    };
    constexpr int kPrefetch = cycle_prefetch_level(D, NOBS, P, (int)sizeof(R));
    MeasurePreloaded<R, D, NOBS, P, kPrefetch, NT> pre{{}, {}, {}, fcov, toff};
    if constexpr (kPrefetch >= 1) {
#pragma unroll
      for (int d = 0; d < D; ++d) pre.mu[d] = packed_load<NTM>(fmean, d, coff);
#pragma unroll
      for (int k = 0; k < NOBS; ++k) pre.ob[k] = packed_load<NTM>(fobs, k, coff);
    }
    if constexpr (kPrefetch >= 2) {
      if (ma.update_cov) {
#pragma unroll
        for (int k = 0; k < P; ++k) pre.cv[k] = packed_load<NT>(fcov, k, toff);
      }
    }
    run_sweeps<R, NR, NC, Energy, CKX, false, GROUP_ALL>(a, en, c, gid, stale_total, x, ledger, total_q5, w, w_r, w_c, fac,
                                                         wave_accepted, bad_energy);
    bad_width |= !(w > R(0));
#pragma unroll
    for (int d = 0; d < D; ++d) fx.store(d, xoff, x[d]);
    if (stale_total) fe.store(Ledger::T, coff, total_q5);
    else ledger.store(fe, coff);
    fw.store(0, coff, w);
    if constexpr (kPrefetch >= 1) {
      measure_chain<R, NR, NC, true, true, NT, NTM>(ma, c, x, pre, fmean, fobs, fcov, ffac, nullptr,
                                                    [&](R &w_real, R &w_cplx) { w_real = w_cplx = w; }, bad_pivot);
    } else {
      const MeasureFromMemory<R, NT, NTM> src{fmean, fobs, fcov, coff, toff};
      measure_chain<R, NR, NC, true, true, NT, NTM>(ma, c, x, src, fmean, fobs, fcov, ffac, nullptr,
                                                    [&](R &w_real, R &w_cplx) { w_real = w_cplx = w; }, bad_pivot);
    }
  }
  if ((threadIdx.x & 63) == 0 && wave_accepted) {
    unsigned long long *slot = a.accept_slots + (size_t)blockIdx.x * (blockDim.x >> 6) + (threadIdx.x >> 6);
    *slot += (unsigned long long)wave_accepted;
  }
  const unsigned int bits = (bad_energy ? ST_NONFINITE_ENERGY : 0u) | (bad_width ? ST_BAD_WIDTH : 0u) | (bad_pivot ? ST_BAD_PIVOT : 0u);
  if (bits) atomicOr(a.status, bits);
}

template <typename R, int NR, int NC, bool NT>
__global__ void __launch_bounds__(kStepThreads) k_factor(const R *cov, R *factor, unsigned int *status, long long n) {
  constexpr int PR = NR * (NR + 1) / 2;
  constexpr int P = PR + NC * NC;
  bool bad_pivot = false;
  const long long stride = (long long)gridDim.x * kStepThreads;
  const TiledField<R> fcov(cov, n, P), ffac(factor, n, P);
  for (long long c = (long long)blockIdx.x * kStepThreads + threadIdx.x; c < n; c += stride) {
    const unsigned int toff = tiled_offset<R>(c, P);
    R m[P];
#pragma unroll
    for (int k = 0; k < P; ++k) m[k] = packed_load<NT>(fcov, k, toff);
#pragma unroll
    for (int i = 0; i < NC; ++i)
#pragma unroll
      for (int j = 0; j < i; ++j) m[cim(PR, i, j)] = -m[cim(PR, i, j)];
    cholesky_packed<R, NR, NC>(m, bad_pivot);
#pragma unroll
    for (int k = 0; k < P; ++k) packed_store<NT>(ffac, k, toff, m[k]);
  }
  if (bad_pivot) atomicOr(status, (unsigned int)ST_BAD_PIVOT);
}

template <typename R, int NR, bool NT>
__global__ void __launch_bounds__(kStepThreads) k_factor_stream(const R *cov, R *factor, unsigned int *status, long long n) {
  constexpr int P = NR * (NR + 1) / 2;
  constexpr int ROWS = sizeof(R) == 4 ? 4 : 2;
  using N_ = Num<R>;
  __shared__ R rows[ROWS][NR][kStepThreads];
  bool bad_pivot = false;
  const long long stride = (long long)gridDim.x * kStepThreads;
  const int lane = threadIdx.x;
  for (long long c = (long long)blockIdx.x * kStepThreads + threadIdx.x; c < n; c += stride) {
    const long long base = (c >> 6) * (long long)P * 64 + (c & 63);
    const R *cv = cov + base;
    R *fc = factor + base;
    for (int i0 = 0; i0 < NR; i0 += ROWS) {
      const int nrows = NR - i0 < ROWS ? NR - i0 : ROWS;
      for (int r = 0; r < nrows; ++r) {
        const R *src = cv + (long long)tri(i0 + r, 0) * 64;
        int j = 0;
        for (; j + 16 <= i0 + r + 1; j += 16) {
          R v[16];
#pragma unroll
          for (int u = 0; u < 16; ++u) v[u] = NT ? __builtin_nontemporal_load(src + (j + u) * 64) : src[(j + u) * 64];
#pragma unroll
          for (int u = 0; u < 16; ++u) rows[r][j + u][lane] = v[u];
        }
        for (; j <= i0 + r; ++j) rows[r][j][lane] = NT ? __builtin_nontemporal_load(src + j * 64) : src[j * 64];
      }
      int j = 0;
      for (; j + 4 <= i0; j += 4) {
        const R *lj[4];
#pragma unroll
        for (int q = 0; q < 4; ++q) lj[q] = fc + (long long)tri(j + q, 0) * 64;
        R s[4][ROWS];
#pragma unroll
        for (int q = 0; q < 4; ++q)
#pragma unroll
          for (int r = 0; r < ROWS; ++r) s[q][r] = R(0);
        int k = 0;
        for (; k + 16 <= j; k += 16) {
          R f[4][16];
// ... 145 lines not shown
```

### metropolisengine_amd/csrc/me_generic.hip

```cpp
#include "me_internal.h"
#include "me_per_device.h"

namespace me {
namespace {

template <typename R>
__global__ void __launch_bounds__(kBlockThreads) k_broadcast_rows(R *dst, const R *row_values, int rows, long long n) {
  const long long stride = (long long)gridDim.x * kBlockThreads;
  for (long long c = (long long)blockIdx.x * kBlockThreads + threadIdx.x; c < n; c += stride)
    for (int r = 0; r < rows; ++r) dst[(long long)r * n + c] = row_values[r];
}

template <typename R>
__global__ void __launch_bounds__(kBlockThreads) k_broadcast_tiled(R *dst, const R *entry_values, int entries, long long n_padded) {
  const long long total = n_padded * entries, stride = (long long)gridDim.x * kBlockThreads;
  for (long long i = (long long)blockIdx.x * kBlockThreads + threadIdx.x; i < total; i += stride)
    dst[i] = entry_values[(i >> 6) % entries];
}

__device__ __forceinline__ void pair_of(int p, int &i, int &j) {
  i = (int)((sqrtf(8.0f * (float)p + 1.0f) - 1.0f) * 0.5f);
  while (i * (i + 1) / 2 > p) --i;
  while ((i + 1) * (i + 2) / 2 <= p) ++i;
  j = p - i * (i + 1) / 2;
}

constexpr int kMaxEntries = 12;

template <typename R, int TILE>
__global__ void __launch_bounds__(kBlockThreads) k_pool_reduce(const R *x, long long n, int nr, int nc, int entry_base, int tiled, double *partials) {
  extern __shared__ __attribute__((aligned(16))) unsigned char smem_raw[];
  R *tile = reinterpret_cast<R *>(smem_raw);
  constexpr int kTilePitch = TILE + 1;
  const int d = nr + 2 * nc;
  const int n_aug = d + nr + nc;
  const int n_pair = d * (d + 1) / 2;
  const int n_entries = 1 + n_aug + n_pair;
  const int tid = threadIdx.x;
  auto at = [&](int r, long long c) -> long long { return tiled ? ((c >> 6) * (long long)d + r) * 64 + (c & 63) : (long long)r * n + c; };

  int row_i[kMaxEntries], row_j[kMaxEntries];
  bool active[kMaxEntries];
  double acc[kMaxEntries];
#pragma unroll
  for (int k = 0; k < kMaxEntries; ++k) {
    const int e = entry_base + tid + k * kBlockThreads;
    acc[k] = 0.0;
    row_i[k] = row_j[k] = -1;
    active[k] = e < n_entries;
    if (!active[k] || e == 0) continue;
    if (e <= n_aug) {
      row_i[k] = e - 1;
    } else {
      pair_of(e - 1 - n_aug, row_i[k], row_j[k]);
    }
  }

  const long long n_tiles = (n + TILE - 1) / TILE;
  for (long long t = blockIdx.x; t < n_tiles; t += gridDim.x) {
    const long long base = t * TILE;
    const int valid = (int)((n - base) < TILE ? (n - base) : TILE);
    for (int r = tid / TILE; r < n_aug; r += kBlockThreads / TILE) {
      const int col = tid % TILE;
      R v = 0;
      if (col < valid) {
        const long long c = base + col;
        if (r < d) v = x[at(r, c)];
        else if (r < d + nr) {
          const R xv = x[at(r - d, c)];
          v = xv < 0 ? -xv : xv;
        } else {
          const int j = r - d - nr;
          const R re = x[at(nr + j, c)], im = x[at(nr + nc + j, c)];
          v = (R)sqrt((double)re * re + (double)im * im);
        }
      }
      tile[r * kTilePitch + col] = v;
    }
    __syncthreads();
#pragma unroll
    for (int k = 0; k < kMaxEntries; ++k) {
      if (!active[k]) continue;
      if (row_i[k] < 0) {
        acc[k] += (double)valid;
      } else if (row_j[k] < 0) {
        const R *ri = tile + row_i[k] * kTilePitch;
        R s = 0;
        for (int col = 0; col < TILE; ++col) s += ri[col];
        acc[k] += (double)s;
      } else {
        const R *ri = tile + row_i[k] * kTilePitch;
        const R *rj = tile + row_j[k] * kTilePitch;
        R s = 0;
        for (int col = 0; col < TILE; ++col) s += ri[col] * rj[col];
        acc[k] += (double)s;
      }
    }
    __syncthreads();
  }
#pragma unroll
  for (int k = 0; k < kMaxEntries; ++k)
    if (active[k]) partials[(long long)blockIdx.x * n_entries + entry_base + tid + k * kBlockThreads] = acc[k];
}

constexpr int kFinishThreads = 1024, kFinishSlices = kFinishThreads / 64;
__global__ void __launch_bounds__(kFinishThreads) k_pool_finish(const double *partials, int n_blocks, int nr, int nc,
                                                                const unsigned long long *slots, long long n_slots,
                                                                double proposed, double *out) {
  const int d = nr + 2 * nc;
  const int n_aug = d + nr + nc;
  const int n_pair = d * (d + 1) / 2;
  const int n_entries = 1 + n_aug + n_pair;
  const int lane = threadIdx.x & 63, slice = threadIdx.x >> 6;
  if (blockIdx.x == gridDim.x - 1) {
    __shared__ unsigned long long wave_sum[kFinishSlices];
    unsigned long long s = 0;
    long long i = threadIdx.x;
    for (; i + 7 * kFinishThreads < n_slots; i += 8 * kFinishThreads) {
      unsigned long long v[8];
#pragma unroll
      for (int u = 0; u < 8; ++u) v[u] = slots[i + u * kFinishThreads];
#pragma unroll
      for (int u = 0; u < 8; ++u) s += v[u];
    }
    for (; i < n_slots; i += kFinishThreads) s += slots[i];
#pragma unroll
    for (int w = 32; w > 0; w >>= 1) s += __shfl_xor(s, w, 64);
    if (lane == 0) wave_sum[slice] = s;
    __syncthreads();
    if (threadIdx.x == 0) {
      unsigned long long t = 0;
#pragma unroll
      for (int w = 0; w < kFinishSlices; ++w) t += wave_sum[w];
      const long long size = moments_size(nr, nc);
      out[size - 2] = (double)t;
      out[size - 1] = proposed;
    }
    return;
  }
  __shared__ double part[kFinishSlices][64];
  const int e = blockIdx.x * 64 + lane;
  double s = 0.0;
  if (e < n_entries) {
#pragma unroll 8
    for (int b = slice; b < n_blocks; b += kFinishSlices) s += partials[(long long)b * n_entries + e];
  }
  part[slice][lane] = s;
  __syncthreads();
  if (slice != 0) return;
  s = 0.0;
#pragma unroll
  for (int w = 0; w < kFinishSlices; ++w) s += part[w][lane];
  if (e == 0) {
    out[0] = s;
  } else if (e <= n_aug) {
    const int r = e - 1;
    out[r < d ? 1 + r : 1 + d + n_pair + (r - d)] = s;
  } else if (e < n_entries) {
    const int p = e - 1 - n_aug;
    int i, j;
    pair_of(p, i, j);
    out[1 + d + p] = s;
    if (i == j && i < nr) out[1 + d + n_pair + nr + nc + i] = s;
  }
}

}

hipError_t launch_broadcast_rows(void *dst, const void *row_values, int rows, long long n, int dtype,
                                 hipStream_t stream) {
  long long blocks = (n + kBlockThreads - 1) / kBlockThreads;
  if (blocks > 4096) blocks = 4096;
  if (blocks < 1) blocks = 1;
  if (dtype == ME_F32)
    hipLaunchKernelGGL(k_broadcast_rows<float>, dim3((unsigned)blocks), dim3(kBlockThreads), 0, stream, (float *)dst,
                       (const float *)row_values, rows, n);
  else
    hipLaunchKernelGGL(k_broadcast_rows<double>, dim3((unsigned)blocks), dim3(kBlockThreads), 0, stream, (double *)dst,
                       (const double *)row_values, rows, n);
  return hipGetLastError();
}

hipError_t launch_broadcast_tiled(void *dst, const void *entry_values, int entries, long long n, int dtype,
                                  hipStream_t stream) {
  const long long n_padded = (n + 63) / 64 * 64;
  long long blocks = (n_padded * entries + kBlockThreads - 1) / kBlockThreads;
  if (blocks > 8192) blocks = 8192;
  if (blocks < 1) blocks = 1;
  if (dtype == ME_F32)
    hipLaunchKernelGGL(k_broadcast_tiled<float>, dim3((unsigned)blocks), dim3(kBlockThreads), 0, stream, (float *)dst,
                       (const float *)entry_values, entries, n_padded);
  else
    hipLaunchKernelGGL(k_broadcast_tiled<double>, dim3((unsigned)blocks), dim3(kBlockThreads), 0, stream, (double *)dst,
                       (const double *)entry_values, entries, n_padded);
  return hipGetLastError();
}

constexpr int kSumThreads = 1024;
__global__ void __launch_bounds__(kSumThreads) k_sum_slots(const unsigned long long *slots, long long n_slots,
                                                           unsigned long long *total) {
  __shared__ unsigned long long part[kSumThreads / 64];
  unsigned long long s = 0;
  long long i = threadIdx.x;
  for (; i + 7 * kSumThreads < n_slots; i += 8 * kSumThreads) {
    unsigned long long v[8];
#pragma unroll
    for (int u = 0; u < 8; ++u) v[u] = slots[i + u * kSumThreads];
#pragma unroll
    for (int u = 0; u < 8; ++u) s += v[u];
  }
  for (; i < n_slots; i += kSumThreads) s += slots[i];
#pragma unroll
  for (int w = 32; w > 0; w >>= 1) s += __shfl_xor(s, w, 64);
  if ((threadIdx.x & 63) == 0) part[threadIdx.x >> 6] = s;
  __syncthreads();
  if (threadIdx.x == 0) {
    unsigned long long t = 0;
#pragma unroll
    for (int w = 0; w < kSumThreads / 64; ++w) t += part[w];
    total[0] = t;
  }
}

template <typename R>
__global__ void __launch_bounds__(kBlockThreads) k_trace(const R *x, const R *energy, const R *width, long long n, int d,
                                                         int n_terms, int width_rows, long long n_traced, long long stride,
                                                         int tiled, double *out) {
  const long long t = (long long)blockIdx.x * kBlockThreads + threadIdx.x;
  if (t >= n_traced) return;
  const long long c = t * stride;
  for (int k = 0; k < d; ++k)
    out[(long long)k * n_traced + t] = (double)x[tiled ? ((c >> 6) * (long long)d + k) * 64 + (c & 63) : (long long)k * n + c];
  for (int k = 0; k < n_terms; ++k) out[(long long)(d + k) * n_traced + t] = (double)energy[(long long)k * n + c];
  for (int r = 0; r < width_rows; ++r)
    out[(long long)(d + n_terms + r) * n_traced + t] = (double)width[(long long)r * n + c];
}

hipError_t launch_trace(const void *x, const void *energy, const void *width, long long n, int d, int n_terms,
                        int width_rows, int dtype, long long n_traced, long long stride, double *out, hipStream_t stream,
                        bool tiled_state) {
  const dim3 grid((unsigned)((n_traced + kBlockThreads - 1) / kBlockThreads)), block(kBlockThreads);
  if (dtype == ME_F32)
    hipLaunchKernelGGL(k_trace<float>, grid, block, 0, stream, (const float *)x, (const float *)energy, (const float *)width,
                       n, d, n_terms, width_rows, n_traced, stride, tiled_state ? 1 : 0, out);
  else
    hipLaunchKernelGGL(k_trace<double>, grid, block, 0, stream, (const double *)x, (const double *)energy,
                       (const double *)width, n, d, n_terms, width_rows, n_traced, stride, tiled_state ? 1 : 0, out);
  return hipGetLastError();
}

hipError_t launch_sum_slots(const unsigned long long *slots, long long n_slots, unsigned long long *total,
                            hipStream_t stream) {
  hipLaunchKernelGGL(k_sum_slots, dim3(1), dim3(kSumThreads), 0, stream, slots, n_slots, total);
  return hipGetLastError();
}

constexpr size_t kPoolLdsLimit = 160 * 1024;
int pool_tile_chains(int nr, int nc, int dtype) {
  const int n_aug = nr + 2 * nc + nr + nc;
  const size_t elem = dtype == ME_F32 ? sizeof(float) : sizeof(double);
  for (int tile : {64, 32, 16})
    if ((size_t)n_aug * (size_t)(tile + 1) * elem <= kPoolLdsLimit) return tile;
  return 0;
}

bool pool_reduce_supported(int nr, int nc, int dtype) { return pool_tile_chains(nr, nc, dtype) != 0; }

int pool_reduce_blocks(long long n, int nr, int nc) {
  const int d = nr + 2 * nc;
  const long long n_entries = 1 + d + nr + nc + (long long)d * (d + 1) / 2;
  long long cap = (32ll << 20) / (8 * n_entries);
  if (cap > 1024) cap = 1024;
  if (cap < 64) cap = 64;
  if (d + nr + nc <= 32) cap = 256;
  const long long tiles = (n + 63) / 64;
  return (int)(tiles < cap ? (tiles < 1 ? 1 : tiles) : cap);
}

namespace {
template <typename R, int TILE>
hipError_t launch_pool_stage1(const void *x, long long n, int nr, int nc, int n_entries, int blocks, double *partials, hipStream_t stream, bool tiled) {
  const size_t lds = (size_t)(nr + 2 * nc + nr + nc) * (size_t)(TILE + 1) * sizeof(R);
  if (lds > 64 * 1024) {
    static PerDevice<hipError_t> attr;
    int device = 0;
    if (hipError_t rc = hipGetDevice(&device); rc != hipSuccess) return rc;
    const hipError_t rc = attr.get(device, [] {
      return hipFuncSetAttribute((const void *)k_pool_reduce<R, TILE>, hipFuncAttributeMaxDynamicSharedMemorySize, (int)kPoolLdsLimit);
    });
    if (rc != hipSuccess) return rc;
  }
  for (int base = 0; base < n_entries; base += kMaxEntries * kBlockThreads)
    hipLaunchKernelGGL((k_pool_reduce<R, TILE>), dim3((unsigned)blocks), dim3(kBlockThreads), lds, stream, (const R *)x, n, nr, nc, base,
                       tiled ? 1 : 0, partials);
  return hipGetLastError();
}
template <typename R>
hipError_t launch_pool_stage1_tile(int tile, const void *x, long long n, int nr, int nc, int n_entries, int blocks, double *partials, hipStream_t stream, bool tiled) {
  switch (tile) {
    case 64: return launch_pool_stage1<R, 64>(x, n, nr, nc, n_entries, blocks, partials, stream, tiled);
    case 32: return launch_pool_stage1<R, 32>(x, n, nr, nc, n_entries, blocks, partials, stream, tiled);
    case 16: return launch_pool_stage1<R, 16>(x, n, nr, nc, n_entries, blocks, partials, stream, tiled);
    default: return hipErrorInvalidValue;
  }
}
}

hipError_t launch_pool_reduce(const void *x, long long n, int nr, int nc, int dtype, const unsigned long long *slots,
                              long long n_slots, double proposed, double *partials, double *out_device,
                              hipStream_t stream,
                              hipError_t (*stage1)(const void *, long long, double *, int, hipStream_t), bool tiled_state) {
  const int d = nr + 2 * nc;
  const int n_aug = d + nr + nc;
  const int n_entries = 1 + n_aug + d * (d + 1) / 2;
  const int tile = pool_tile_chains(nr, nc, dtype);
  if (!stage1 && tile == 0) return hipErrorInvalidValue;
  const int blocks = pool_reduce_blocks(n, nr, nc);
  hipError_t err;
  if (stage1) err = stage1(x, n, partials, blocks, stream);
  else if (dtype == ME_F32) err = launch_pool_stage1_tile<float>(tile, x, n, nr, nc, n_entries, blocks, partials, stream, tiled_state);
  else err = launch_pool_stage1_tile<double>(tile, x, n, nr, nc, n_entries, blocks, partials, stream, tiled_state);
  if (err != hipSuccess) return err;
  hipLaunchKernelGGL(k_pool_finish, dim3((unsigned)((n_entries + 63) / 64 + 1)), dim3(kFinishThreads), 0, stream,
                     (const double *)partials, blocks, nr, nc, slots, n_slots, proposed, out_device);
  return hipGetLastError();
}

}
```

### metropolisengine_amd/csrc/me_internal.h

```cpp
#pragma once

#include <hip/hip_runtime.h>
#include <stdint.h>

#include "../../include/metropolis_engine.h"

namespace me {

enum CovKind { CK_IDENTITY = 0, CK_SHARED = 1, CK_PER_CHAIN = 2, CK_PER_CHAIN_NT = 3 };

enum StepGroup { GROUP_ALL = 0, GROUP_REAL = 1, GROUP_COMPLEX = 2 };

enum StatusBits : uint32_t {
  ST_NONFINITE_ENERGY = 1u,
  ST_BAD_PIVOT = 2u,
  ST_BAD_WIDTH = 4u
};

long long cache_budget_bytes();
void set_cache_budget_bytes(long long bytes);

constexpr int kBlockThreads = 256;
#ifndef ME_STEP_THREADS
#define ME_STEP_THREADS 64
#endif
constexpr int kStepThreads = ME_STEP_THREADS;
constexpr int kFusedStepThreads = 256;
constexpr int kFusedSweepsThreshold = 4;

struct StepLaunch {
  int n_real, n_complex;
  void *x, *energy, *width;
  const void *factor;
  const void *factor_full;
  const void *factor_image;
  const void *energy_image;
  const void *coef_device;
  const double *coef_host;
  int n_coef;
  const void *inj_normals;
  const void *inj_uniforms;
  unsigned long long *accept_slots;
  unsigned int *status;
  long long n;
  unsigned long long chain_offset, step_index, seed;
  int n_sweeps, energy_kind, cov_kind, reject_kind, grid_blocks;
  int group;
  int split_widths;
  int stale_total;
  const void *cov;
  double reject_bound, temp, ratio, target_acceptance, damping;
};

struct MeasureLaunch {
  int n_real, n_complex;
  void *x, *width, *mean, *cov, *obs_mean, *factor;
  unsigned int *status;
  long long n;
  unsigned long long measure_count;
  int update_cov;
  int split_widths;
  int write_factor;
  int grid_blocks;
};

struct EnergyLaunch {
  int n_real, n_complex;
  int total_row;
  void *x, *energy;
  const void *coef_device;
  const double *coef_host;
  int n_coef;
  unsigned int *status;
  long long n;
  int energy_kind, grid_blocks;
};

constexpr int kMaxRegisterDof = 96;

struct KernelSet {
  const char *user_name;
  int dtype, n_real, n_complex;
  bool per_chain_cov;
  bool tracks_cov;
  bool (*has_energy)(int energy_kind);
  int (*energy_terms)(int energy_kind);
  hipError_t (*step)(const StepLaunch &, hipStream_t);
  hipError_t (*magphase)(const StepLaunch &, hipStream_t);
  hipError_t (*measure)(const MeasureLaunch &, hipStream_t);
  hipError_t (*init_energy)(const EnergyLaunch &, hipStream_t);
  size_t matrix_image_bytes;
  hipError_t (*prepare_matrix)(const void *matrix, void *image, hipStream_t);
  hipError_t (*pool_stage1)(const void *x, long long n, double *partials, int n_rows, hipStream_t);
  bool has_user_reject;
  bool streams_packed;
  hipError_t (*cycle)(const StepLaunch &, const MeasureLaunch &, hipStream_t);
  bool tiled_state;
};

void register_kernel_set(const KernelSet *set);
const KernelSet *find_kernel_set(int dtype, int n_real, int n_complex, int energy_kind, const char *user_name);
bool has_dims(int dtype, int n_real, int n_complex);

hipError_t launch_broadcast_rows(void *dst, const void *row_values, int rows, long long n, int dtype,
                                 hipStream_t stream);
hipError_t launch_broadcast_tiled(void *dst, const void *entry_values, int entries, long long n, int dtype,
                                  hipStream_t stream);
hipError_t launch_pool_reduce(const void *x, long long n, int n_real, int n_complex, int dtype,
                              const unsigned long long *slots, long long n_slots, double proposed, double *partials,
                              double *out_device, hipStream_t stream,
                              hipError_t (*stage1)(const void *, long long, double *, int, hipStream_t) = nullptr,
                              bool tiled_state = false);
int pool_reduce_blocks(long long n, int n_real, int n_complex);
bool pool_reduce_supported(int n_real, int n_complex, int dtype);
hipError_t launch_trace(const void *x, const void *energy, const void *width, long long n, int d, int n_terms,
                        int width_rows, int dtype, long long n_traced, long long stride, double *out, hipStream_t stream,
                        bool tiled_state = false);
hipError_t launch_detect_equilibration(const double *series, long long n_series, long long length, int fast, int nskip,
                                       double *scratch, long long *t0_out, double *g_out, double *neff_out,
                                       hipStream_t stream);
hipError_t launch_sum_slots(const unsigned long long *slots, long long n_slots, unsigned long long *total,
                            hipStream_t stream);

inline int grid_for(long long n, int requested, int threads = kStepThreads) {
  long long blocks = (n + threads - 1) / threads;
  if (requested > 0 && blocks > requested) blocks = requested;
  if (blocks < 1) blocks = 1;
  return (int)blocks;
}

__host__ __device__ inline int packed_real(int nr) { return nr * (nr + 1) / 2; }
__host__ __device__ inline int packed_total(int nr, int nc) { return nr * (nr + 1) / 2 + nc * nc; }
__host__ __device__ inline int n_observables(int nr, int nc) { return 2 * nr + nc; }
__host__ __device__ inline long long moments_size(int nr, int nc) {
  const int d = nr + 2 * nc;
  return 1 + d + (long long)d * (d + 1) / 2 + n_observables(nr, nc) + 2;
}

}
```

### metropolisengine_amd/csrc/me_kernels.hip

```cpp
#include <type_traits>

#include "me_device.h"
#include "me_dense_mfma.h"
#include "me_dense_bf16x3.h"
#include "me_dense_f64.h"
#include "me_factor_tile.h"
#include "me_per_device.h"
#include "me_pool_gram.h"
#include "me_magphase.h"

#ifdef ME_USER_SOURCE
#include ME_USER_SOURCE
#endif

#ifndef ME_NR
#error "compile with -DME_NR=<n_real> -DME_NC=<n_complex>"
#endif
#ifndef ME_DENSE
#define ME_DENSE 0
#endif
#ifndef ME_PER_CHAIN
#define ME_PER_CHAIN 1
#endif
#ifndef ME_TRACK_COV
// ... 46 lines not shown
__device__ R me_user_energy_entry(const R *x, const R *coef) { return me_user_energy<R>(x, coef); }
__device__ user_fn_t<float> g_user_fn_f32 = &me_user_energy_entry<float>;
__device__ user_fn_t<double> g_user_fn_f64 = &me_user_energy_entry<double>;
template <typename R, int NR_, int NC_>
struct EnergyUserIndirect {
  static constexpr int D = NR_ + 2 * NC_;
  user_fn_t<R> fn;
  const R *coef;
  __device__ __forceinline__ R operator()(const R (&x)[D]) const { return fn(x, coef); }
#ifdef ME_USER_HAS_REJECT
  __device__ __forceinline__ bool reject(const R (&x)[D]) const { return me_user_reject<R>(x, coef); }
#endif
};
template <typename R>
user_fn_t<R> load_user_fn() {
  user_fn_t<R> fn = nullptr;
  if constexpr (std::is_same<R, float>::value) (void)hipMemcpyFromSymbol(&fn, HIP_SYMBOL(g_user_fn_f32), sizeof(fn));
  else (void)hipMemcpyFromSymbol(&fn, HIP_SYMBOL(g_user_fn_f64), sizeof(fn));
  return fn;
}
#endif

int energy_terms(int kind) {
#ifdef ME_USER_SOURCE
#ifdef ME_USER_N_TERMS
  if (kind == ME_ENERGY_USER) return ME_USER_N_TERMS;
#else
  if (kind == ME_ENERGY_USER) return 1;
#endif
  return kind == ME_ENERGY_USER_INDIRECT ? 1 : 0;
#endif
  switch (kind) {
    case ME_ENERGY_ISO_QUAD:
    case ME_ENERGY_DIAG_QUAD: return 1;
    case ME_ENERGY_DENSE_QUAD: return ME_DENSE != 0 ? 1 : 0;
    case ME_ENERGY_LANDAU_TOY: return kLandau ? 1 : 0;
    case ME_ENERGY_LANDAU_TERMS: return kLandau ? 2 : 0;
    case ME_ENERGY_CYLINDER: return kCylinder ? 1 : 0;
    default: return 0;
  }
}
bool has_energy(int kind) { return energy_terms(kind) > 0; }

template <typename R>
StepArgs<R> typed(const StepLaunch &l) {
  StepArgs<R> a;
  a.x = (R *)l.x;
  a.energy = (R *)l.energy;
  a.width = (R *)l.width;
  a.factor = (const R *)l.factor;
  a.inj_normals = (const R *)l.inj_normals;
  a.inj_uniforms = (const R *)l.inj_uniforms;
  a.accept_slots = l.accept_slots;
  a.status = l.status;
  a.n = l.n;
  a.chain_offset = l.chain_offset;
  a.step_index = l.step_index;
  a.seed_lo = (uint32_t)l.seed;
  a.seed_hi = (uint32_t)(l.seed >> 32);
  a.n_sweeps = l.n_sweeps;
  a.reject_kind = l.reject_kind;
  a.split_widths = l.split_widths;
  a.stale_total = l.stale_total;
  a.reject_bound = (R)l.reject_bound;
  a.temp = (R)l.temp;
  a.inv_temp = l.temp > 0 ? (R)(1.0 / l.temp) : (R)0;
  a.inv_temp_log2e = l.temp > 0 ? (R)(1.4426950408889634 / l.temp) : (R)0;
  a.ratio = (R)l.ratio;
  a.p = (R)l.target_acceptance;
  a.damping = (R)l.damping;
  a.up = (R)(l.ratio * (1.0 - l.target_acceptance) / l.damping);
  a.down = (R)(-l.ratio * l.target_acceptance / l.damping);
  return a;
}

template <typename R, class Energy, bool INJECT, int GROUP>
hipError_t launch_step_cov(const StepLaunch &l, const StepArgs<R> &a, const Energy &en, dim3 grid, dim3 block,
                           hipStream_t stream) {
  switch (l.cov_kind) {
    case CK_IDENTITY: {
      constexpr long long state_bytes = (long long)sizeof(R) * (D + 2);
      if constexpr (!INJECT && GROUP == GROUP_ALL) {
        if (state_bytes * l.n > 2 * cache_budget_bytes()) {
          hipLaunchKernelGGL((k_step<R, NR, NC, Energy, CK_IDENTITY, INJECT, GROUP, true>), grid, block, 0, stream, a, en);
          break;
        }
      }
      hipLaunchKernelGGL((k_step<R, NR, NC, Energy, CK_IDENTITY, INJECT, GROUP>), grid, block, 0, stream, a, en);
      break;
    }
    case CK_SHARED: hipLaunchKernelGGL((k_step<R, NR, NC, Energy, CK_SHARED, INJECT, GROUP>), grid, block, 0, stream, a, en); break;
#if ME_PER_CHAIN == 2
    case CK_PER_CHAIN: {
      if constexpr (INJECT) return hipErrorInvalidValue;
      else hipLaunchKernelGGL((k_step<R, NR, NC, Energy, CK_PER_CHAIN_NT, INJECT, GROUP>), grid, block, 0, stream, a, en);
      break;
    }
#elif ME_PER_CHAIN
    case CK_PER_CHAIN: {
      constexpr long long per_chain_bytes = (long long)sizeof(R) * (D + 2 + NR * (NR + 1) / 2 + NC * NC);
      if constexpr (!INJECT) {
        if (per_chain_bytes * l.n > cache_budget_bytes()) {
          hipLaunchKernelGGL((k_step<R, NR, NC, Energy, CK_PER_CHAIN_NT, INJECT, GROUP>), grid, block, 0, stream, a, en);
          break;
        }
      }
      hipLaunchKernelGGL((k_step<R, NR, NC, Energy, CK_PER_CHAIN, INJECT, GROUP>), grid, block, 0, stream, a, en);
      break;
    }
#endif
    default: return hipErrorInvalidValue;
  }
  return hipGetLastError();
}

template <typename R, class Energy, bool INJECT>
hipError_t launch_step_group(const StepLaunch &l, const StepArgs<R> &a, const Energy &en, dim3 grid, dim3 block,
                             hipStream_t stream) {
  if (l.group == GROUP_ALL) return launch_step_cov<R, Energy, INJECT, GROUP_ALL>(l, a, en, grid, block, stream);
  if constexpr (NR > 0 && NC > 0) {
    if (l.group == GROUP_REAL) return launch_step_cov<R, Energy, INJECT, GROUP_REAL>(l, a, en, grid, block, stream);
    if (l.group == GROUP_COMPLEX) return launch_step_cov<R, Energy, INJECT, GROUP_COMPLEX>(l, a, en, grid, block, stream);
  }
  return hipErrorInvalidValue;
}

template <typename R, class Energy>
hipError_t step_with(const StepLaunch &l, const Energy &en, hipStream_t stream) {
  const StepArgs<R> a = typed<R>(l);
  const bool per_chain = l.cov_kind == CK_PER_CHAIN;
  const int threads = (l.n_sweeps >= kFusedSweepsThreshold || (ME_PER_CHAIN == 2 && per_chain)) ? kFusedStepThreads : kStepThreads;
  const dim3 grid(grid_for(l.n, l.grid_blocks, threads)), block(threads);
  if (l.inj_normals) {
    if constexpr (std::is_same<R, double>::value) return launch_step_group<R, Energy, true>(l, a, en, grid, block, stream);
    else return hipErrorNotSupported;
  }
#if ME_DENSE && !defined(ME_USER_SOURCE)
  if constexpr (std::is_same<R, float>::value && NR == 64 && NC == 0 &&
                std::is_same<Energy, EnergyDense<float, 64, 0>>::value) {
    if (per_chain) return launch_step_group<R, Energy, false>(l, a, en, grid, block, stream);
    if (dense64_exact_fp32_mfma()) {
      if (l.cov_kind == CK_IDENTITY)
        return launch_step_dense64_mfma<CK_IDENTITY>(a, en.a, nullptr, l.grid_blocks, stream);
      if (l.cov_kind == CK_SHARED && l.factor_full)
        return launch_step_dense64_mfma<CK_SHARED>(a, en.a, (const float *)l.factor_full, l.grid_blocks, stream);
      return hipErrorInvalidValue;
    }
    if (!l.energy_image) return hipErrorInvalidValue;
    if (l.cov_kind == CK_IDENTITY)
      return launch_step_dense64_bf16x3<CK_IDENTITY>(a, (const unsigned int *)l.energy_image, nullptr, l.grid_blocks, stream);
    if (l.cov_kind == CK_SHARED && l.factor_image)
      return launch_step_dense64_bf16x3<CK_SHARED>(a, (const unsigned int *)l.energy_image,
                                                   (const unsigned int *)l.factor_image, l.grid_blocks, stream);
    return hipErrorInvalidValue;
  } else if constexpr (std::is_same<R, double>::value && NR == 64 && NC == 0 &&
                       std::is_same<Energy, EnergyDense<double, 64, 0>>::value) {
    if (per_chain) return launch_step_group<R, Energy, false>(l, a, en, grid, block, stream);
    if (!l.energy_image) return hipErrorInvalidValue;
    if (l.cov_kind == CK_IDENTITY)
      return launch_step_dense64_f64<CK_IDENTITY>(a, (const double *)l.energy_image, nullptr, l.grid_blocks, stream);
    if (l.cov_kind == CK_SHARED && l.factor_image)
      return launch_step_dense64_f64<CK_SHARED>(a, (const double *)l.energy_image, (const double *)l.factor_image,
                                                l.grid_blocks, stream);
    return hipErrorInvalidValue;
  } else
#endif
    return launch_step_group<R, Energy, false>(l, a, en, grid, block, stream);
}

template <typename R, class Energy>
hipError_t magphase_with(const StepLaunch &l, const Energy &en, hipStream_t stream) {
#if ME_PER_CHAIN
  if constexpr (NC > 0) {
    StepArgs<R> a = typed<R>(l);
    a.factor = (const R *)l.cov;
    const dim3 grid(grid_for(l.n, l.grid_blocks)), block(kStepThreads);
    if (l.inj_normals) {
      if constexpr (std::is_same<R, double>::value)
        hipLaunchKernelGGL((k_step_magphase<R, NR, NC, Energy, true>), grid, block, 0, stream, a, en);
      else
        return hipErrorNotSupported;
    } else {
      hipLaunchKernelGGL((k_step_magphase<R, NR, NC, Energy, false>), grid, block, 0, stream, a, en);
    }
    return hipGetLastError();
  }
#endif
  return hipErrorNotSupported;
}

// ... 54 lines not shown
    case ME_ENERGY_CYLINDER: {
      if constexpr (kCylinder) {
        if (n_coef != 3) return hipErrorInvalidValue;
        EnergyCylinder<R, NR, NC> en{(R)coef[0], (R)coef[1], (R)coef[2]};
        return f(en);
      }
      return hipErrorInvalidValue;
    }
    default: return hipErrorInvalidValue;
  }
#endif
}

template <typename R>
hipError_t step(const StepLaunch &l, hipStream_t stream) {
  return with_energy<R>(l.energy_kind, l.coef_host, l.n_coef, l.coef_device,
                        [&](const auto &en) { return step_with<R>(l, en, stream); });
}

template <typename R>
hipError_t magphase(const StepLaunch &l, hipStream_t stream) {
  return with_energy<R>(l.energy_kind, l.coef_host, l.n_coef, l.coef_device,
                        [&](const auto &en) { return magphase_with<R>(l, en, stream); });
}

template <typename R>
hipError_t init_energy(const EnergyLaunch &l, hipStream_t stream) {
  return with_energy<R>(l.energy_kind, l.coef_host, l.n_coef, l.coef_device, [&](const auto &en) {
    using Energy = std::decay_t<decltype(en)>;
    hipLaunchKernelGGL((k_init_energy<R, NR, NC, Energy>), dim3(grid_for(l.n, l.grid_blocks)), dim3(kStepThreads), 0,
                       stream, (const R *)l.x, (R *)l.energy, l.n, l.status, en, l.total_row);
    return hipGetLastError();
  });
}

template <typename R>
MeasureArgs<R> typed_measure(const MeasureLaunch &l) {
  MeasureArgs<R> a;
  a.x = (const R *)l.x;
  a.width = (const R *)l.width;
  a.mean = (R *)l.mean;
  a.cov = (R *)l.cov;
  a.obs_mean = (R *)l.obs_mean;
  a.factor = (R *)l.factor;
  a.status = l.status;
  a.n = l.n;
  const double i = (double)l.measure_count;
  a.keep = (R)((i - 1.0) / i);
  a.inv_i = (R)(1.0 / i);
  a.cov_keep = (R)((i - 2.0) / (i - 1.0));
  a.update_cov = l.update_cov;
  a.split_widths = l.split_widths;
  a.write_factor = l.write_factor;
  return a;
}

#ifndef ME_FACTOR_TILE
#define ME_FACTOR_TILE 1
#endif
#ifndef ME_CYCLE
#define ME_CYCLE (ME_PER_CHAIN == 1)
#endif
template <typename R>
hipError_t cycle(const StepLaunch &l, const MeasureLaunch &ml, hipStream_t stream) {
#if ME_CYCLE
  constexpr int P = NR * (NR + 1) / 2 + NC * NC;
  if constexpr (P <= kMaxPackedInRegisters) {
    if (l.group != GROUP_ALL || l.inj_normals || !ml.cov || !ml.factor) return hipErrorNotSupported;
    if (l.cov_kind != CK_IDENTITY && l.cov_kind != CK_PER_CHAIN) return hipErrorNotSupported;
    return with_energy<R>(l.energy_kind, l.coef_host, l.n_coef, l.coef_device, [&](const auto &en) -> hipError_t {
      using Energy = std::decay_t<decltype(en)>;
#if ME_DENSE && !defined(ME_USER_SOURCE)
      if constexpr (NR == 64 && NC == 0 && std::is_same<Energy, EnergyDense<R, 64, 0>>::value) return hipErrorNotSupported;
#endif
      const StepArgs<R> a = typed<R>(l);
      const MeasureArgs<R> ma = typed_measure<R>(ml);
      constexpr long long mean_bytes = (long long)sizeof(R) * (2 * D + (2 * NR + NC));
      constexpr long long all_bytes = mean_bytes + (long long)sizeof(R) * (2 + 2 * P);
      const bool nt = all_bytes * l.n > cache_budget_bytes(), ntm = mean_bytes * l.n > cache_budget_bytes();
      const int threads = l.n_sweeps >= kFusedSweepsThreshold ? kFusedStepThreads : kStepThreads;
      const dim3 grid(grid_for(l.n, l.grid_blocks, threads)), block(threads);
      auto launch = [&](auto ck) {
        constexpr int CK = decltype(ck)::value;
        if (ntm) hipLaunchKernelGGL((k_cycle<R, NR, NC, Energy, CK, true, true>), grid, block, 0, stream, a, ma, en);
        else if (nt) hipLaunchKernelGGL((k_cycle<R, NR, NC, Energy, CK, true, false>), grid, block, 0, stream, a, ma, en);
        else hipLaunchKernelGGL((k_cycle<R, NR, NC, Energy, CK, false, false>), grid, block, 0, stream, a, ma, en);
      };
      if (l.cov_kind == CK_PER_CHAIN) launch(std::integral_constant<int, CK_PER_CHAIN>{});
      else launch(std::integral_constant<int, CK_IDENTITY>{});
      return hipGetLastError();
    });
  }
#endif
  return hipErrorNotSupported;
}

template <typename R>
hipError_t measure(const MeasureLaunch &l, hipStream_t stream) {
  const MeasureArgs<R> a = typed_measure<R>(l);
  constexpr int P = NR * (NR + 1) / 2 + NC * NC;
  constexpr bool kFused = ME_PER_CHAIN == 1 && P <= ME_MEASURE_FUSED_MAX_P;
  const dim3 grid(grid_for(l.n, l.grid_blocks)), block(kStepThreads);
  constexpr long long mean_bytes = (long long)sizeof(R) * (2 * D + (2 * NR + NC));
  constexpr long long all_bytes = mean_bytes + (long long)sizeof(R) * 2 * P;
  const bool nt = all_bytes * l.n > cache_budget_bytes(), ntm = mean_bytes * l.n > cache_budget_bytes();
  constexpr bool kCov = (ME_PER_CHAIN != 0 || ME_TRACK_COV != 0);
  if (l.cov) {
    if (ntm) hipLaunchKernelGGL((k_measure<R, NR, NC, kCov, kFused, true, true>), grid, block, 0, stream, a);
    else if (nt) hipLaunchKernelGGL((k_measure<R, NR, NC, kCov, kFused, true, false>), grid, block, 0, stream, a);
    else hipLaunchKernelGGL((k_measure<R, NR, NC, kCov, kFused, false, false>), grid, block, 0, stream, a);
  } else {
    if (ntm) hipLaunchKernelGGL((k_measure<R, NR, NC, false, false, false, true>), grid, block, 0, stream, a);
    else hipLaunchKernelGGL((k_measure<R, NR, NC, false, false, false, false>), grid, block, 0, stream, a);
  }
#if ME_PER_CHAIN == 1
  if constexpr (!kFused) {
    if (l.update_cov && l.write_factor) {
      if (nt) hipLaunchKernelGGL((k_factor<R, NR, NC, true>), grid, block, 0, stream, (const R *)l.cov, (R *)l.factor, l.status, l.n);
      else hipLaunchKernelGGL((k_factor<R, NR, NC, false>), grid, block, 0, stream, (const R *)l.cov, (R *)l.factor, l.status, l.n);
    }
  }
#elif ME_PER_CHAIN == 2
  static_assert(P > kMaxPackedInRegisters, "ME_PER_CHAIN=2 is for spaces with more than 160 packed entries");
  if (l.cov && l.update_cov && l.write_factor) {
    if constexpr (NC > 0) {
      if (nt) hipLaunchKernelGGL((k_factor_mixed<R, NR, NC, true>), grid, block, 0, stream, (const R *)l.cov, (R *)l.factor, l.status, l.n);
      else hipLaunchKernelGGL((k_factor_mixed<R, NR, NC, false>), grid, block, 0, stream, (const R *)l.cov, (R *)l.factor, l.status, l.n);
    } else if constexpr (NR <= 64 && ME_FACTOR_TILE) {
      const hipError_t err = nt ? launch_factor_tile<R, NR, true>((const R *)l.cov, (R *)l.factor, l.status, l.n, stream)
                                : launch_factor_tile<R, NR, false>((const R *)l.cov, (R *)l.factor, l.status, l.n, stream);
      if (err != hipSuccess) return err;
    } else {
      if (nt) hipLaunchKernelGGL((k_factor_stream<R, NR, true>), grid, block, 0, stream, (const R *)l.cov, (R *)l.factor, l.status, l.n);
      else hipLaunchKernelGGL((k_factor_stream<R, NR, false>), grid, block, 0, stream, (const R *)l.cov, (R *)l.factor, l.status, l.n);
    }
  }
#endif
  return hipGetLastError();
}

#ifdef ME_USER_SOURCE
#define ME_SET_NAME ME_USER_NAME
#else
#define ME_SET_NAME nullptr
#endif
constexpr auto pool_stage1_f32() -> hipError_t (*)(const void *, long long, double *, int, hipStream_t) {
  if constexpr (NR == 64 && NC == 0) return launch_pool_gram64;
  else if constexpr (D + NR + NC <= 32) return launch_pool_gram32<NR, NC>;
  else return nullptr;
}
constexpr auto pool_stage1_f64() -> hipError_t (*)(const void *, long long, double *, int, hipStream_t) {
  if constexpr (NR == 64 && NC == 0) return launch_pool_gram64_f64;
  else if constexpr (D + NR + NC <= 32) return launch_pool_gram32_f64<NR, NC>;
  else return nullptr;
}
#if ME_DENSE && !defined(ME_USER_SOURCE)
hipError_t prepare_matrix_f32(const void *factor_full, void *image, hipStream_t stream) {
  if constexpr (NR == 64 && NC == 0) {
    hipLaunchKernelGGL(k_dense64_bf16_fragments<0>, dim3(1), dim3(256), 0, stream, (const float *)factor_full,
                       (unsigned int *)image);
    return hipGetLastError();
  }
  return hipSuccess;
}
[[maybe_unused]] constexpr size_t kMatrixImageBytes = (NR == 64 && NC == 0) ? sizeof(unsigned int) * kBf16FragWords : 0;
#define ME_PREPARE_MATRIX_F32 kMatrixImageBytes, (kMatrixImageBytes ? prepare_matrix_f32 : nullptr), pool_stage1_f32()
hipError_t prepare_matrix_f64(const void *matrix, void *image, hipStream_t stream) {
  if constexpr (NR == 64 && NC == 0) {
    hipLaunchKernelGGL(k_dense64_f64_fragments<0>, dim3(1), dim3(256), 0, stream, (const double *)matrix, (double *)image);
    return hipGetLastError();
  }
  return hipSuccess;
}
[[maybe_unused]] constexpr size_t kMatrixImageBytesF64 = (NR == 64 && NC == 0) ? sizeof(double) * kDense64F64ImageDoubles : 0;
#define ME_PREPARE_MATRIX_F64 kMatrixImageBytesF64, (kMatrixImageBytesF64 ? prepare_matrix_f64 : nullptr), pool_stage1_f64()
#else
#define ME_PREPARE_MATRIX_F32 0, nullptr, pool_stage1_f32()
#define ME_PREPARE_MATRIX_F64 0, nullptr, pool_stage1_f64()
#endif
#ifdef ME_USER_HAS_REJECT
constexpr bool kHasUserReject = true;
#else
constexpr bool kHasUserReject = false;
#endif
#ifndef ME_ONLY_DTYPE
#define ME_ONLY_DTYPE 0
#endif
#if ME_ONLY_DTYPE != 64
const KernelSet kSetF32 = {ME_SET_NAME, ME_F32, NR, NC, ME_PER_CHAIN != 0, (ME_PER_CHAIN != 0 || ME_TRACK_COV != 0), has_energy, energy_terms, step<float>,
                           (NC > 0 && ME_PER_CHAIN == 1) ? magphase<float> : nullptr, measure<float>, init_energy<float>,
                           ME_PREPARE_MATRIX_F32, kHasUserReject, ME_PER_CHAIN == 2, cycle<float>, D >= kTiledStateDof};
#endif
#if ME_ONLY_DTYPE != 32
const KernelSet kSetF64 = {ME_SET_NAME, ME_F64, NR, NC, ME_PER_CHAIN != 0, (ME_PER_CHAIN != 0 || ME_TRACK_COV != 0), has_energy, energy_terms, step<double>,
                           (NC > 0 && ME_PER_CHAIN == 1) ? magphase<double> : nullptr, measure<double>, init_energy<double>,
                           ME_PREPARE_MATRIX_F64, kHasUserReject, ME_PER_CHAIN == 2, cycle<double>, D >= kTiledStateDof};
#endif

struct Registrar {
  Registrar() {
#if ME_ONLY_DTYPE != 64
    register_kernel_set(&kSetF32);
#endif
#if ME_ONLY_DTYPE != 32
    register_kernel_set(&kSetF64);
#endif
  }
} registrar;

}
}
```

### metropolisengine_amd/csrc/me_magphase.h

```cpp
#pragma once

#include "me_device.h"

namespace me {

template <typename R>
struct Trig;
template <>
struct Trig<float> {
  static __device__ __forceinline__ void unit_phase(float u, float &c, float &s) {
    c = __builtin_amdgcn_cosf(u - 0.5f);
    s = __builtin_amdgcn_sinf(u - 0.5f);
  }
};
template <>
struct Trig<double> {
  static __device__ __forceinline__ void unit_phase(double u, double &c, double &s) {
    const double theta = -3.141592653589793 + 6.283185307179586 * u;
    c = cos(theta);
    s = sin(theta);
  }
};

template <typename R, int NR, int NC, class Energy, bool INJECT = false>
__global__ void __launch_bounds__(kStepThreads) k_step_magphase(StepArgs<R> a, Energy en) {
  static_assert(NC > 0, "the magnitude-phase sampler acts on complex parameters");
  constexpr int D = NR + 2 * NC;
  constexpr int PR = NR * (NR + 1) / 2;
  constexpr int P = PR + NC * NC;
  constexpr int W1 = 2 * ((NC + 1) / 2);
  constexpr int NWORDS = W1 + NC + 2;
  constexpr int NBLK = (NWORDS + 3) / 4;
  constexpr bool MIXED = NR > 0;
  constexpr int WROW = MIXED ? GROUP_COMPLEX : 0;
  using N_ = Num<R>;

  if constexpr (!INJECT) N_::prepare();
  energy_prepare(en, 0);
  unsigned int wave_accepted = 0;
  bool bad_energy = false, bad_width = false;
  const long long stride = (long long)gridDim.x * kStepThreads;
  using Ledger = EnergyLedger<R, Energy, MIXED ? GROUP_COMPLEX : GROUP_ALL>;
  const XField<R, D> fx(a.x, a.n);
  const Field<R> fe(a.energy, a.n, Ledger::T), fw(a.width, a.n, MIXED ? 3 : 1);
  const TiledField<R> fcov(a.factor, a.n, P);
  for (long long c = (long long)blockIdx.x * kStepThreads + threadIdx.x; c < a.n; c += stride) {
    const unsigned int coff = (unsigned int)c * (unsigned int)sizeof(R);
    const unsigned int xoff = fx.offset(c);
    R x[D], kdiag[NC];
#pragma unroll
    for (int d = 0; d < D; ++d) x[d] = fx.load(d, xoff);
#pragma unroll
    for (int j = 0; j < NC; ++j) kdiag[j] = fcov.load(cdiag(PR, j), tiled_offset<R>(c, P));
    Ledger ledger;
    ledger.load(fe, coff);
    R w = fw.load(WROW, coff);
    const unsigned long long gid = a.chain_offset + (unsigned long long)c;

    auto decide = [&](const R (&xp)[D], R u) -> bool {
      bool rejected = false;
      if (a.reject_kind == ME_REJECT_ABS_REAL0_GE) rejected = !(N_::abs_(xp[0]) < a.reject_bound);
      else if (a.reject_kind == ME_REJECT_USER) rejected = energy_reject(en, xp, 0);
      R terms_new[Ledger::T];
      const R e_new = ledger.propose(en, xp, terms_new);
      const R diff = e_new - ledger.partial();
      bool accept = diff <= R(0);
      if (a.temp > R(0)) accept = accept || N_::uphill(u, diff, a.inv_temp, a.inv_temp_log2e);
      accept = accept && !rejected;
      bad_energy |= (!rejected && !N_::finite(e_new));
#pragma unroll
      for (int d = NR; d < D; ++d) x[d] = accept ? xp[d] : x[d];
      ledger.commit(accept, terms_new);
      wave_accepted += (unsigned int)__popcll(__ballot(accept));
      return accept;
    };

    for (int s = 0; s < a.n_sweeps; ++s) {
      const unsigned long long step = a.step_index + (unsigned long long)s;
      R g[W1], u_mag, u_phase[NC], u_ph;
      if constexpr (INJECT) {
#pragma unroll
        for (int j = 0; j < NC; ++j) g[j] = a.inj_normals[((long long)s * NC + j) * a.n + c];
        u_mag = a.inj_uniforms[((long long)s * (NC + 2) + 0) * a.n + c];
#pragma unroll
        for (int j = 0; j < NC; ++j) u_phase[j] = a.inj_uniforms[((long long)s * (NC + 2) + 1 + j) * a.n + c];
        u_ph = a.inj_uniforms[((long long)s * (NC + 2) + NC + 1) * a.n + c];
      } else {
        uint32_t words[4 * NBLK];
#pragma unroll
        for (int b = 0; b < NBLK; ++b) {
          U4 ctr;
          ctr.x = (uint32_t)gid;
          ctr.y = (uint32_t)(gid >> 32);
          ctr.z = (uint32_t)step;
          ctr.w = ((uint32_t)(step >> 32) << 16) | (uint32_t)b;
          const U4 o = philox4x32_10(ctr, a.seed_lo, a.seed_hi);
          words[4 * b + 0] = o.x;
          words[4 * b + 1] = o.y;
          words[4 * b + 2] = o.z;
          words[4 * b + 3] = o.w;
        }
#pragma unroll
        for (int q = 0; q < W1 / 2; ++q) N_::normal_pair(words[2 * q], words[2 * q + 1], g[2 * q], g[2 * q + 1]);
        u_mag = N_::unit(words[W1]);
#pragma unroll
        for (int j = 0; j < NC; ++j) u_phase[j] = N_::unit(words[W1 + 1 + j]);
        u_ph = N_::unit(words[W1 + NC + 1]);
      }

      R xp[D];
#pragma unroll
      for (int d = 0; d < D; ++d) xp[d] = x[d];
#pragma unroll
      for (int j = 0; j < NC; ++j) {
        const R re = x[NR + j], im = x[NR + NC + j];
        const R mag = N_::sqrt_(re * re + im * im);
        const R inv = mag > R(0) ? R(1) / mag : R(0);
        const R dre = mag > R(0) ? re * inv : R(1);
        const R dim = mag > R(0) ? im * inv : R(0);
        const R mnew = mag + (w * w * kdiag[j]) * g[j];
        xp[NR + j] = mnew * dre;
        xp[NR + NC + j] = mnew * dim;
      }
      const bool acc_mag = decide(xp, u_mag);
      w = N_::adapt(w, acc_mag, a.ratio, a.p, a.damping, a.up, a.down);
#pragma unroll
      for (int j = 0; j < NC; ++j) {
        const R re = x[NR + j], im = x[NR + NC + j];
        const R mag = N_::sqrt_(re * re + im * im);
        R cs, sn;
        Trig<R>::unit_phase(u_phase[j], cs, sn);
        xp[NR + j] = mag * cs;
        xp[NR + NC + j] = mag * sn;
      }
// ... 18 lines not shown
```

Baseline: 19.64 billion.

## Store f64 chain state as contiguous per-chain records with vector buffer loads

Adds a chain-major state layout for f64 kernels with 8 to 63 parameters (a multiple of 8). Each chain's parameter vector becomes a contiguous record, loaded and stored with 128-bit buffer operations instead of one strided load per component. Stores happen only for chains whose state moved. When most lanes in a wave moved, the stores are staged through LDS so the wave writes coalesced tiles. Host copy, broadcast, trace and pool paths are generalised to the new layout, at the cost of extra LDS use and per-lane access patterns that are less coalesced than tile-major.

```diff
diff --git a/metropolisengine_amd/csrc/me_api.hip b/metropolisengine_amd/csrc/me_api.hip
--- a/metropolisengine_amd/csrc/me_api.hip
+++ b/metropolisengine_amd/csrc/me_api.hip
@@ -148,7 +148,7 @@
   unsigned long long *accept_slots = nullptr, *accept_total = nullptr;
   long long n_slots = 0;
   unsigned long long proposed = 0;
-  bool x_tiled = false;
+  int x_layout = STATE_COMPONENT_MAJOR;
   int width_rows = 1;
   bool widths_synced = true;
   unsigned int *status = nullptr;
@@ -190,28 +190,28 @@
   }
 }
 
-int broadcast(me_engine *e, void *dst, const std::vector<double> &row, bool tiled = false) {
+int broadcast(me_engine *e, void *dst, const std::vector<double> &row, int tile_chains = 0) {
   std::vector<unsigned char> bytes;
   to_device_type(row.data(), row.size(), e->dtype, bytes);
   ME_HIP(e, hipMemcpyAsync(e->row_dev, bytes.data(), bytes.size(), hipMemcpyHostToDevice, e->stream));
-  if (tiled) ME_HIP(e, launch_broadcast_tiled(dst, e->row_dev, (int)row.size(), e->n, e->dtype, e->stream));
+  if (tile_chains > 0) ME_HIP(e, launch_broadcast_tiled(dst, e->row_dev, (int)row.size(), e->n, e->dtype, e->stream, tile_chains));
   else ME_HIP(e, launch_broadcast_rows(dst, e->row_dev, (int)row.size(), e->n, e->dtype, e->stream));
   ME_HIP(e, hipStreamSynchronize(e->stream));
   return ME_OK;
 }
 
 int check_status(me_engine *e);
-int copy_tiled(me_engine *e, void *field_ptr, int entries, int64_t chain_begin, int64_t n_chains, double *dst, const double *src) {
-  const int64_t tile0 = chain_begin >> 6, tile1 = (chain_begin + n_chains - 1) >> 6;
-  const size_t tile_values = (size_t)entries * 64, n_values = (size_t)(tile1 - tile0 + 1) * tile_values;
-  unsigned char *dev = (unsigned char *)field_ptr + (size_t)tile0 * tile_values * e->esize;
-  std::vector<unsigned char> tmp(n_values * e->esize);
-  const bool whole = (chain_begin & 63) == 0 && (((chain_begin + n_chains) & 63) == 0 || chain_begin + n_chains == e->n);
-  if (dst || !whole) {
+int copy_tiled(me_engine *e, void *field_ptr, int entries, int64_t chain_begin, int64_t n_chains, double *dst, const double *src,
+               int tile_chains = 64) {
+  const TileSpan span = tile_span(chain_begin, n_chains, tile_chains, e->n);
+  const size_t tile_values = (size_t)entries * tile_chains;
+  unsigned char *dev = (unsigned char *)field_ptr + (size_t)span.first_tile * tile_values * e->esize;
+  std::vector<unsigned char> tmp((size_t)span.n_tiles * tile_values * e->esize);
+  if (dst || !span.whole) {
     ME_HIP(e, hipMemcpyAsync(tmp.data(), dev, tmp.size(), hipMemcpyDeviceToHost, e->stream));
     ME_HIP(e, hipStreamSynchronize(e->stream));
   }
-  auto at = [&](int64_t c, int k) { return (size_t)((c >> 6) - tile0) * tile_values + (size_t)k * 64 + (size_t)(c & 63); };
+  auto at = [&](int64_t c, int k) { return tiled_index(c, k, entries, tile_chains, span.first_tile); };
   if (e->dtype == ME_F32) {
     float *t = reinterpret_cast<float *>(tmp.data());
     for (int64_t i = 0; i < n_chains; ++i)
@@ -507,8 +507,8 @@
   ME_CREATE_HIP(hipStreamCreateWithFlags(&e->stream, hipStreamNonBlocking));
   e->own_stream = true;
   const size_t n = (size_t)e->n, es = e->esize;
-  e->x_tiled = ks->tiled_state;
-  ME_CREATE_HIP(hipMalloc(&e->x, (e->x_tiled ? (n + 63) / 64 * 64 : n) * e->d * es));
+  e->x_layout = ks->state_layout;
+  ME_CREATE_HIP(hipMalloc(&e->x, (e->x_layout != STATE_COMPONENT_MAJOR ? (n + 63) / 64 * 64 : n) * e->d * es));
   e->stale_total = (c->flags & ME_FLAG_REFERENCE_ENERGY_LEDGERS) != 0;
   ME_CREATE_HIP(hipMalloc(&e->energy, n * (e->n_terms + (e->stale_total ? 1 : 0)) * es));
   e->width_rows = (e->nr > 0 && e->nc > 0) ? 3 : 1;
@@ -615,9 +615,10 @@
   }
   int rc = ME_OK;
   std::vector<double> width_row((size_t)e->width_rows, c->sampling_width);
-  if ((rc = broadcast(e, e->x, init, e->x_tiled)) || (rc = broadcast(e, e->mean, init)) || (rc = broadcast(e, e->obs_mean, obs)) ||
-      (rc = broadcast(e, e->width, width_row)) || (e->cov && (rc = broadcast(e, e->cov, c0, true))) ||
-      (e->factor && (rc = broadcast(e, e->factor, f0, true)))) {
+  const int x_tile = e->x_layout == STATE_COMPONENT_MAJOR ? 0 : state_tile_chains(e->x_layout);
+  if ((rc = broadcast(e, e->x, init, x_tile)) || (rc = broadcast(e, e->mean, init)) || (rc = broadcast(e, e->obs_mean, obs)) ||
+      (rc = broadcast(e, e->width, width_row)) || (e->cov && (rc = broadcast(e, e->cov, c0, 64))) ||
+      (e->factor && (rc = broadcast(e, e->factor, f0, 64)))) {
     g_create_error = e->err;
     release(e);
     return rc;
@@ -669,7 +670,7 @@
     return fail(e, ME_ERR_UNSUPPORTED, is_user_kind(energy_kind)
                     ? std::string("no user-energy plugin named '") + (user_name ? user_name : "") + "' is loaded for these dimensions"
                     : "energy kind " + std::to_string(energy_kind) + " is not compiled for these dimensions");
-  if (ks->tiled_state != e->ks->tiled_state || ks->per_chain_cov != e->ks->per_chain_cov || ks->streams_packed != e->ks->streams_packed ||
+  if (ks->state_layout != e->ks->state_layout || ks->per_chain_cov != e->ks->per_chain_cov || ks->streams_packed != e->ks->streams_packed ||
       ks->tracks_cov != e->ks->tracks_cov)
     return fail(e, ME_ERR_UNSUPPORTED, "me_set_energy: the plugin was built with other per-chain covariance options than this engine's kernel set");
   if (e->reject_kind == ME_REJECT_USER && !ks->has_user_reject)
@@ -881,7 +882,7 @@
     }
     const int rows_valid = (e->width_rows == 3 && e->widths_synced) ? 1 : e->width_rows;
     ME_HIP(e, launch_trace(e->x, e->energy, e->width, e->n, e->d, e->n_terms, rows_valid, e->dtype, e->trace_chains, e->trace_stride,
-                           e->trace_dev + e->trace_rows * cols * e->trace_chains, e->stream, e->x_tiled));
+                           e->trace_dev + e->trace_rows * cols * e->trace_chains, e->stream, e->x_layout));
     if (rows_valid != e->width_rows) {
       double *row = e->trace_dev + e->trace_rows * cols * e->trace_chains + (size_t)(e->d + e->n_terms) * e->trace_chains;
       for (int r = 1; r < 3; ++r)
@@ -991,8 +992,9 @@
   int rc = field_info(e, field, &ptr, &comps);
   if (rc != ME_OK) return rc;
   if (n_chains == 0) return ME_OK;
-  if (field == ME_FIELD_COV || field == ME_FIELD_FACTOR || (field == ME_FIELD_PARAMS && e->x_tiled))
-    return copy_tiled(e, ptr, comps, chain_begin, n_chains, dst, nullptr);
+  if (field == ME_FIELD_COV || field == ME_FIELD_FACTOR) return copy_tiled(e, ptr, comps, chain_begin, n_chains, dst, nullptr);
+  if (field == ME_FIELD_PARAMS && e->x_layout != STATE_COMPONENT_MAJOR)
+    return copy_tiled(e, ptr, comps, chain_begin, n_chains, dst, nullptr, state_tile_chains(e->x_layout));
   std::vector<unsigned char> tmp((size_t)comps * n_chains * e->esize);
   for (int r = 0; r < comps; ++r)
     ME_HIP(e, hipMemcpyAsync(tmp.data() + (size_t)r * n_chains * e->esize,
@@ -1024,8 +1026,9 @@
   if (field == ME_FIELD_WIDTH && e->width_rows == 3 && (chain_begin != 0 || n_chains != e->n))
     return fail(e, ME_ERR_INVALID, "widths of a mixed engine must be set for all chains at once");
   if (n_chains == 0) return ME_OK;
-  if (field == ME_FIELD_COV || field == ME_FIELD_FACTOR || (field == ME_FIELD_PARAMS && e->x_tiled)) {
-    rc = copy_tiled(e, ptr, comps, chain_begin, n_chains, nullptr, src);
+  if (field == ME_FIELD_COV || field == ME_FIELD_FACTOR || (field == ME_FIELD_PARAMS && e->x_layout != STATE_COMPONENT_MAJOR)) {
+    rc = copy_tiled(e, ptr, comps, chain_begin, n_chains, nullptr, src,
+                    field == ME_FIELD_PARAMS ? state_tile_chains(e->x_layout) : 64);
     if (rc != ME_OK) return rc;
     if (field == ME_FIELD_FACTOR) e->cov_kind = CK_PER_CHAIN;
     return ME_OK;
@@ -1111,7 +1114,7 @@
   ME_HIP(e, hipSetDevice(e->device));
   hipError_t err = launch_pool_reduce(e->x, e->n, e->nr, e->nc, e->dtype, e->accept_slots, e->n_slots,
                                       (double)e->proposed, e->pool_partials, (double *)device_out, e->stream,
-                                      e->ks->pool_stage1, e->x_tiled);
+                                      e->ks->pool_stage1, e->x_layout);
   if (err == hipErrorInvalidValue) return fail(e, ME_ERR_UNSUPPORTED, "pooled moments: dimension too large for the reduction kernel");
   ME_HIP(e, err);
   return ME_OK;
diff --git a/metropolisengine_amd/csrc/me_device.h b/metropolisengine_amd/csrc/me_device.h
--- a/metropolisengine_amd/csrc/me_device.h
+++ b/metropolisengine_amd/csrc/me_device.h
@@ -217,13 +217,92 @@
 #define ME_TILED_STATE_DOF 16
 #endif
 constexpr int kTiledStateDof = ME_TILED_STATE_DOF;
+#ifndef ME_STATE_LAYOUT
+#define ME_STATE_LAYOUT STATE_CHAIN_MAJOR
+#endif
+template <typename R, int D>
+constexpr int state_layout_of() {
+  if (D < kTiledStateDof) return STATE_COMPONENT_MAJOR;
+  if (ME_STATE_LAYOUT == STATE_CHAIN_MAJOR && sizeof(R) == 8 && D < 64 && D % 8 == 0) return STATE_CHAIN_MAJOR;
+  return STATE_TILE_MAJOR;
+}
+template <typename R, bool NT>
+struct RecordField {
+  static_assert(sizeof(R) == 8, "chain-major records are float64");
+  typedef unsigned int V4 __attribute__((ext_vector_type(4)));
+  typedef unsigned int V2 __attribute__((ext_vector_type(2)));
+  typedef R R2 __attribute__((ext_vector_type(2)));
+  static constexpr int kAux = NT ? ME_NT_AUX : 0;
+  __amdgpu_buffer_rsrc_t rsrc;
+  __device__ __forceinline__ RecordField(const R *base, long long n, int entries)
+      : rsrc(__builtin_amdgcn_make_buffer_rsrc(const_cast<R *>(base), 0,
+                                               (unsigned int)(((n + 63) >> 6) * 64 * (long long)entries * (long long)sizeof(R)),
+                                               0x00020000)) {}
+  __device__ __forceinline__ R load(int row, unsigned int off) const {
+    return __builtin_bit_cast(R, __builtin_amdgcn_raw_buffer_load_b64(rsrc, off, (unsigned int)row * 8u, kAux));
+  }
+  __device__ __forceinline__ void store(int row, unsigned int off, R value) const {
+    __builtin_amdgcn_raw_buffer_store_b64(__builtin_bit_cast(V2, value), rsrc, off, (unsigned int)row * 8u, kAux);
+  }
+  template <int D>
+  __device__ __forceinline__ void load_record(R (&x)[D], unsigned int off) const {
+#pragma unroll
+    for (int q = 0; q < D / 2; ++q) {
+      const R2 v = __builtin_bit_cast(R2, __builtin_amdgcn_raw_buffer_load_b128(rsrc, off, (unsigned int)q * 16u, kAux));
+      x[2 * q] = v.x;
+      x[2 * q + 1] = v.y;
+    }
+  }
+  template <int D>
+  __device__ __forceinline__ void store_record(const R (&x)[D], unsigned int off) const {
+#pragma unroll
+    for (int q = 0; q < D / 2; ++q)
+      __builtin_amdgcn_raw_buffer_store_b128(__builtin_bit_cast(V4, R2{x[2 * q], x[2 * q + 1]}), rsrc, off, (unsigned int)q * 16u, kAux);
+  }
+  template <int K>
+  static __device__ __forceinline__ unsigned int slot(unsigned int l, unsigned int q) {
+    if constexpr (K % 8 == 0) return l * K + (q ^ ((l >> 1) & 7u));
+    else return l * K + q;
+  }
+  template <int D>
+  __device__ __forceinline__ void store_tile(const R (&x)[D], unsigned int off, bool write, V4 *slab) const {
+    constexpr int K = D / 2;
+    const unsigned int lane = threadIdx.x & 63u;
+    const unsigned int tile_off = off - lane * (unsigned int)(D * sizeof(R));
+#pragma unroll
+    for (int q = 0; q < K; ++q) slab[slot<K>(lane, q)] = __builtin_bit_cast(V4, R2{x[2 * q], x[2 * q + 1]});
+    asm volatile("s_waitcnt lgkmcnt(0)" ::: "memory");
+    const int w = write ? 1 : 0;
+#pragma unroll
+    for (int i = 0; i < K; ++i) {
+      const unsigned int p = (unsigned int)i * 64u + lane, l = p / K, q = slot<K>(l, p % K) - l * K;
+      if (__builtin_amdgcn_ds_bpermute((int)(l * 4u), w))
+        __builtin_amdgcn_raw_buffer_store_b128(slab[p], rsrc, tile_off + l * (unsigned int)(D * sizeof(R)) + q * 16u, 0u, kAux);
+      __builtin_amdgcn_sched_barrier(0);
+    }
+  }
+};
+template <typename R, int D>
+constexpr bool record_tile_stores() {
+  return state_layout_of<R, D>() == STATE_CHAIN_MAJOR && (kFusedStepThreads / 64) * 64 * D * (int)sizeof(R) <= 32768;
+}
+template <typename R, int D>
+constexpr size_t record_store_lds_bytes(unsigned int threads) {
+  return record_tile_stores<R, D>() ? (size_t)(threads / 64) * 64 * D * sizeof(R) : 0;
+}
+#ifndef ME_TILE_STORE_MIN_MOVED
+#define ME_TILE_STORE_MIN_MOVED 43
+#endif
 template <typename R, int D, bool NTS = false>
 struct XField {
-  static constexpr bool kTiled = D >= kTiledStateDof;
-  std::conditional_t<kTiled, TiledField<R>, StateField<R, NTS>> f;
+  static constexpr int kLayout = state_layout_of<R, D>();
+  static constexpr bool kTiled = kLayout == STATE_TILE_MAJOR;
+  static constexpr bool kRecords = kLayout == STATE_CHAIN_MAJOR;
+  std::conditional_t<kRecords, RecordField<R, NTS>, std::conditional_t<kTiled, TiledField<R>, StateField<R, NTS>>> f;
   __device__ __forceinline__ XField(const R *base, long long n) : f(base, n, D) {}
   static __device__ __forceinline__ unsigned int offset(long long c) {
     if constexpr (kTiled) return tiled_offset<R>(c, D);
+    else if constexpr (kRecords) return (unsigned int)c * (unsigned int)(D * sizeof(R));
     else return (unsigned int)c * (unsigned int)sizeof(R);
   }
   __device__ __forceinline__ R load(int row, unsigned int off) const {
@@ -234,11 +313,40 @@
     if constexpr (kTiled && NTS) f.store_nt(row, off, value);
     else f.store(row, off, value);
   }
+  __device__ __forceinline__ void load_all(R (&x)[D], unsigned int off) const {
+    if constexpr (kRecords) {
+      f.load_record(x, off);
+    } else {
+#pragma unroll
+      for (int d = 0; d < D; ++d) x[d] = load(d, off);
+    }
+  }
+  __device__ __forceinline__ void store_all(const R (&x)[D], unsigned int off) const {
+    if constexpr (kRecords) {
+      f.store_record(x, off);
+    } else {
+#pragma unroll
+      for (int d = 0; d < D; ++d) store(d, off, x[d]);
+    }
+  }
+  __device__ __forceinline__ void store_moved(const R (&x)[D], unsigned int off, bool moved, [[maybe_unused]] void *lds) const {
+    if constexpr (!kRecords) {
+      store_all(x, off);
+    } else {
+      if constexpr (record_tile_stores<R, D>()) {
+        if (__ballot(true) == ~0ull && __popcll(__ballot(moved)) > ME_TILE_STORE_MIN_MOVED) {
+          using V4 = typename RecordField<R, NTS>::V4;
+          f.store_tile(x, off, moved, reinterpret_cast<V4 *>(lds) + (threadIdx.x >> 6) * 64 * (D / 2));
+          return;
+        }
+      }
+      if (moved) f.store_record(x, off);
+    }
+  }
 };
 template <typename R, int D>
 __device__ __forceinline__ long long state_index(long long c, int row, long long n) {
-  if constexpr (D >= kTiledStateDof) return ((c >> 6) * (long long)D + row) * 64 + (c & 63);
-  else return (long long)row * n + c;
+  return state_offset(state_layout_of<R, D>(), c, row, D, n);
 }
 
 constexpr int kMaxPackedInRegisters = 160;
@@ -590,7 +698,7 @@
 __device__ __forceinline__ void decide_step(const StepArgs<R> &a, const Energy &en, bool stale_total, R u,
                                             const R (&g)[2 * ((NR + 2 * NC + 1) / 2)], R (&x)[NR + 2 * NC], const R (&xp)[NR + 2 * NC],
                                             Ledger &ledger, R &total_q5, R &w, R &w_r, R &w_c, unsigned int &wave_accepted,
-                                            bool &bad_energy) {
+                                            bool &moved, bool &bad_energy) {
   [[maybe_unused]] constexpr int D = NR + 2 * NC;
   constexpr bool MOVE_REAL = NR > 0 && GROUP != GROUP_COMPLEX;
   constexpr bool MOVE_COMPLEX = NC > 0 && GROUP != GROUP_REAL;
@@ -628,20 +736,21 @@
   if constexpr (GROUP == GROUP_ALL) w_r = w_c = w;
   else if constexpr (GROUP == GROUP_REAL) w_r = w;
   else w_c = w;
+  moved |= accept;
   wave_accepted += (unsigned int)__popcll(__ballot(accept));
 }
 
 template <typename R, int NR, int NC, class Energy, int CK, bool INJECT, int GROUP, class Ledger, class Fac>
 __device__ __forceinline__ void run_sweeps(const StepArgs<R> &a, const Energy &en, long long c, unsigned long long gid,
                                            bool stale_total, R (&x)[NR + 2 * NC], Ledger &ledger, R &total_q5, R &w, R &w_r,
-                                           R &w_c, Fac &&fac, unsigned int &wave_accepted, bool &bad_energy) {
+                                           R &w_c, Fac &&fac, unsigned int &wave_accepted, bool &moved, bool &bad_energy) {
   constexpr int D = NR + 2 * NC;
   constexpr int NW = 2 * ((D + 1) / 2);
   for (int s = 0; s < a.n_sweeps; ++s) {
     R g[NW], u, xp[D];
     draw_step<R, NR, NC, INJECT>(a, c, gid, s, g, u);
     propose_registers<R, NR, NC, CK, GROUP>(x, g, w_r, w_c, fac, xp);
-    decide_step<R, NR, NC, Energy, CK, GROUP>(a, en, stale_total, u, g, x, xp, ledger, total_q5, w, w_r, w_c, wave_accepted, bad_energy);
+    decide_step<R, NR, NC, Energy, CK, GROUP>(a, en, stale_total, u, g, x, xp, ledger, total_q5, w, w_r, w_c, wave_accepted, moved, bad_energy);
   }
 }
 
@@ -670,6 +779,7 @@
 
 template <typename R, int NR, int NC, class Energy, int CK, bool INJECT = false, int GROUP = GROUP_ALL, bool NTS = false>
 __global__ void ME_STEP_BOUNDS k_step(StepArgs<R> a, Energy en) {
+  extern __shared__ __attribute__((aligned(16))) unsigned char step_lds[];
   constexpr int D = NR + 2 * NC;
   constexpr bool MIXED = NR > 0 && NC > 0;
   static_assert(GROUP == GROUP_ALL || MIXED, "group-wise kernels exist for mixed engines only");
@@ -694,8 +804,8 @@
     const unsigned int coff = (unsigned int)c * (unsigned int)sizeof(R);
     const unsigned int xoff = fx.offset(c);
     R x[D];
-#pragma unroll
-    for (int d = 0; d < D; ++d) x[d] = fx.load(d, xoff);
+    fx.load_all(x, xoff);
+    bool moved = false;
     Ledger ledger;
     R total_q5 = R(0);
     if (stale_total) total_q5 = fe.load(Ledger::T, coff);
@@ -824,14 +934,14 @@
         if constexpr (GROUP == GROUP_ALL) w_r = w_c = w;
         else if constexpr (GROUP == GROUP_REAL) w_r = w;
         else w_c = w;
+        moved |= accept;
         wave_accepted += (unsigned int)__popcll(__ballot(accept));
       }
     } else {
-      run_sweeps<R, NR, NC, Energy, CK, INJECT, GROUP>(a, en, c, gid, stale_total, x, ledger, total_q5, w, w_r, w_c, fac, wave_accepted, bad_energy);
+      run_sweeps<R, NR, NC, Energy, CK, INJECT, GROUP>(a, en, c, gid, stale_total, x, ledger, total_q5, w, w_r, w_c, fac, wave_accepted, moved, bad_energy);
     }
     bad_width |= !(w > R(0));
-#pragma unroll
-    for (int d = 0; d < D; ++d) fx.store(d, xoff, x[d]);
+    fx.store_moved(x, xoff, moved, step_lds);
     if (stale_total) fe.store(Ledger::T, coff, total_q5);
     else ledger.store(fe, coff);
     fw.store(MIXED ? GROUP : 0, coff, w);
@@ -1119,8 +1229,7 @@
     const unsigned int coff = (unsigned int)c * (unsigned int)sizeof(R);
     const unsigned int xoff = fx.offset(c);
     R x[D];
-#pragma unroll
-    for (int d = 0; d < D; ++d) x[d] = fx.load(d, xoff);
+    fx.load_all(x, xoff);
     const MeasureFromMemory<R, NT, NTM> src{fmean, fobs, fcov, coff, tiled_offset<R>(c, P)};
     measure_chain<R, NR, NC, PER_CHAIN_COV, FUSED, NT, NTM>(a, c, x, src, fmean, fobs, fcov, ffac, s_delta, [&](R &w_real, R &w_cplx) {
       constexpr bool MIXED = NR > 0 && NC > 0;
@@ -1138,6 +1247,7 @@
 
 template <typename R, int NR, int NC, class Energy, int CK, bool NT, bool NTM>
 __global__ void ME_STEP_BOUNDS k_cycle(StepArgs<R> a, MeasureArgs<R> ma, Energy en) {
+  extern __shared__ __attribute__((aligned(16))) unsigned char step_lds[];
   constexpr int D = NR + 2 * NC;
   constexpr int P = NR * (NR + 1) / 2 + NC * NC;
   constexpr int NOBS = 2 * NR + NC;
@@ -1161,8 +1271,8 @@
     const unsigned int coff = (unsigned int)c * (unsigned int)sizeof(R);
     const unsigned int xoff = fx.offset(c);
     R x[D];
-#pragma unroll
-    for (int d = 0; d < D; ++d) x[d] = fx.load(d, xoff);
+    fx.load_all(x, xoff);
+    bool moved = false;
     Ledger ledger;
     R total_q5 = R(0);
     if (stale_total) total_q5 = fe.load(Ledger::T, coff);
@@ -1196,10 +1306,9 @@
       }
     }
     run_sweeps<R, NR, NC, Energy, CKX, false, GROUP_ALL>(a, en, c, gid, stale_total, x, ledger, total_q5, w, w_r, w_c, fac,
-                                                         wave_accepted, bad_energy);
+                                                         wave_accepted, moved, bad_energy);
     bad_width |= !(w > R(0));
-#pragma unroll
-    for (int d = 0; d < D; ++d) fx.store(d, xoff, x[d]);
+    fx.store_moved(x, xoff, moved, step_lds);
     if (stale_total) fe.store(Ledger::T, coff, total_q5);
     else ledger.store(fe, coff);
     fw.store(0, coff, w);
diff --git a/metropolisengine_amd/csrc/me_generic.hip b/metropolisengine_amd/csrc/me_generic.hip
--- a/metropolisengine_amd/csrc/me_generic.hip
+++ b/metropolisengine_amd/csrc/me_generic.hip
@@ -12,10 +12,11 @@
 }
 
 template <typename R>
-__global__ void __launch_bounds__(kBlockThreads) k_broadcast_tiled(R *dst, const R *entry_values, int entries, long long n_padded) {
+__global__ void __launch_bounds__(kBlockThreads) k_broadcast_tiled(R *dst, const R *entry_values, int entries, long long n_padded,
+                                                                   int tile_chains) {
   const long long total = n_padded * entries, stride = (long long)gridDim.x * kBlockThreads;
   for (long long i = (long long)blockIdx.x * kBlockThreads + threadIdx.x; i < total; i += stride)
-    dst[i] = entry_values[(i >> 6) % entries];
+    dst[i] = entry_values[(i / tile_chains) % entries];
 }
 
 __device__ __forceinline__ void pair_of(int p, int &i, int &j) {
@@ -28,7 +29,7 @@
 constexpr int kMaxEntries = 12;
 
 template <typename R, int TILE>
-__global__ void __launch_bounds__(kBlockThreads) k_pool_reduce(const R *x, long long n, int nr, int nc, int entry_base, int tiled, double *partials) {
+__global__ void __launch_bounds__(kBlockThreads) k_pool_reduce(const R *x, long long n, int nr, int nc, int entry_base, int layout, double *partials) {
   extern __shared__ __attribute__((aligned(16))) unsigned char smem_raw[];
   R *tile = reinterpret_cast<R *>(smem_raw);
   constexpr int kTilePitch = TILE + 1;
@@ -37,7 +38,7 @@
   const int n_pair = d * (d + 1) / 2;
   const int n_entries = 1 + n_aug + n_pair;
   const int tid = threadIdx.x;
-  auto at = [&](int r, long long c) -> long long { return tiled ? ((c >> 6) * (long long)d + r) * 64 + (c & 63) : (long long)r * n + c; };
+  auto at = [&](int r, long long c) -> long long { return state_offset(layout, c, r, d, n); };
 
   int row_i[kMaxEntries], row_j[kMaxEntries];
   bool active[kMaxEntries];
@@ -182,17 +183,17 @@
 }
 
 hipError_t launch_broadcast_tiled(void *dst, const void *entry_values, int entries, long long n, int dtype,
-                                  hipStream_t stream) {
+                                  hipStream_t stream, int tile_chains) {
   const long long n_padded = (n + 63) / 64 * 64;
   long long blocks = (n_padded * entries + kBlockThreads - 1) / kBlockThreads;
   if (blocks > 8192) blocks = 8192;
   if (blocks < 1) blocks = 1;
   if (dtype == ME_F32)
     hipLaunchKernelGGL(k_broadcast_tiled<float>, dim3((unsigned)blocks), dim3(kBlockThreads), 0, stream, (float *)dst,
-                       (const float *)entry_values, entries, n_padded);
+                       (const float *)entry_values, entries, n_padded, tile_chains);
   else
     hipLaunchKernelGGL(k_broadcast_tiled<double>, dim3((unsigned)blocks), dim3(kBlockThreads), 0, stream, (double *)dst,
-                       (const double *)entry_values, entries, n_padded);
+                       (const double *)entry_values, entries, n_padded, tile_chains);
   return hipGetLastError();
 }
 
@@ -225,12 +226,12 @@
 template <typename R>
 __global__ void __launch_bounds__(kBlockThreads) k_trace(const R *x, const R *energy, const R *width, long long n, int d,
                                                          int n_terms, int width_rows, long long n_traced, long long stride,
-                                                         int tiled, double *out) {
+                                                         int layout, double *out) {
   const long long t = (long long)blockIdx.x * kBlockThreads + threadIdx.x;
   if (t >= n_traced) return;
   const long long c = t * stride;
   for (int k = 0; k < d; ++k)
-    out[(long long)k * n_traced + t] = (double)x[tiled ? ((c >> 6) * (long long)d + k) * 64 + (c & 63) : (long long)k * n + c];
+    out[(long long)k * n_traced + t] = (double)x[state_offset(layout, c, k, d, n)];
   for (int k = 0; k < n_terms; ++k) out[(long long)(d + k) * n_traced + t] = (double)energy[(long long)k * n + c];
   for (int r = 0; r < width_rows; ++r)
     out[(long long)(d + n_terms + r) * n_traced + t] = (double)width[(long long)r * n + c];
@@ -238,14 +239,14 @@
 
 hipError_t launch_trace(const void *x, const void *energy, const void *width, long long n, int d, int n_terms,
                         int width_rows, int dtype, long long n_traced, long long stride, double *out, hipStream_t stream,
-                        bool tiled_state) {
+                        int state_layout) {
   const dim3 grid((unsigned)((n_traced + kBlockThreads - 1) / kBlockThreads)), block(kBlockThreads);
   if (dtype == ME_F32)
     hipLaunchKernelGGL(k_trace<float>, grid, block, 0, stream, (const float *)x, (const float *)energy, (const float *)width,
-                       n, d, n_terms, width_rows, n_traced, stride, tiled_state ? 1 : 0, out);
+                       n, d, n_terms, width_rows, n_traced, stride, state_layout, out);
   else
     hipLaunchKernelGGL(k_trace<double>, grid, block, 0, stream, (const double *)x, (const double *)energy,
-                       (const double *)width, n, d, n_terms, width_rows, n_traced, stride, tiled_state ? 1 : 0, out);
+                       (const double *)width, n, d, n_terms, width_rows, n_traced, stride, state_layout, out);
   return hipGetLastError();
 }
 
@@ -279,7 +280,7 @@
 
 namespace {
 template <typename R, int TILE>
-hipError_t launch_pool_stage1(const void *x, long long n, int nr, int nc, int n_entries, int blocks, double *partials, hipStream_t stream, bool tiled) {
+hipError_t launch_pool_stage1(const void *x, long long n, int nr, int nc, int n_entries, int blocks, double *partials, hipStream_t stream, int layout) {
   const size_t lds = (size_t)(nr + 2 * nc + nr + nc) * (size_t)(TILE + 1) * sizeof(R);
   if (lds > 64 * 1024) {
     static PerDevice<hipError_t> attr;
@@ -292,15 +293,15 @@
   }
   for (int base = 0; base < n_entries; base += kMaxEntries * kBlockThreads)
     hipLaunchKernelGGL((k_pool_reduce<R, TILE>), dim3((unsigned)blocks), dim3(kBlockThreads), lds, stream, (const R *)x, n, nr, nc, base,
-                       tiled ? 1 : 0, partials);
+                       layout, partials);
   return hipGetLastError();
 }
 template <typename R>
-hipError_t launch_pool_stage1_tile(int tile, const void *x, long long n, int nr, int nc, int n_entries, int blocks, double *partials, hipStream_t stream, bool tiled) {
+hipError_t launch_pool_stage1_tile(int tile, const void *x, long long n, int nr, int nc, int n_entries, int blocks, double *partials, hipStream_t stream, int layout) {
   switch (tile) {
-    case 64: return launch_pool_stage1<R, 64>(x, n, nr, nc, n_entries, blocks, partials, stream, tiled);
-    case 32: return launch_pool_stage1<R, 32>(x, n, nr, nc, n_entries, blocks, partials, stream, tiled);
-    case 16: return launch_pool_stage1<R, 16>(x, n, nr, nc, n_entries, blocks, partials, stream, tiled);
+    case 64: return launch_pool_stage1<R, 64>(x, n, nr, nc, n_entries, blocks, partials, stream, layout);
+    case 32: return launch_pool_stage1<R, 32>(x, n, nr, nc, n_entries, blocks, partials, stream, layout);
+    case 16: return launch_pool_stage1<R, 16>(x, n, nr, nc, n_entries, blocks, partials, stream, layout);
     default: return hipErrorInvalidValue;
   }
 }
@@ -309,7 +310,7 @@
 hipError_t launch_pool_reduce(const void *x, long long n, int nr, int nc, int dtype, const unsigned long long *slots,
                               long long n_slots, double proposed, double *partials, double *out_device,
                               hipStream_t stream,
-                              hipError_t (*stage1)(const void *, long long, double *, int, hipStream_t), bool tiled_state) {
+                              hipError_t (*stage1)(const void *, long long, double *, int, hipStream_t), int state_layout) {
   const int d = nr + 2 * nc;
   const int n_aug = d + nr + nc;
   const int n_entries = 1 + n_aug + d * (d + 1) / 2;
@@ -318,8 +319,8 @@
   const int blocks = pool_reduce_blocks(n, nr, nc);
   hipError_t err;
   if (stage1) err = stage1(x, n, partials, blocks, stream);
-  else if (dtype == ME_F32) err = launch_pool_stage1_tile<float>(tile, x, n, nr, nc, n_entries, blocks, partials, stream, tiled_state);
-  else err = launch_pool_stage1_tile<double>(tile, x, n, nr, nc, n_entries, blocks, partials, stream, tiled_state);
+  else if (dtype == ME_F32) err = launch_pool_stage1_tile<float>(tile, x, n, nr, nc, n_entries, blocks, partials, stream, state_layout);
+  else err = launch_pool_stage1_tile<double>(tile, x, n, nr, nc, n_entries, blocks, partials, stream, state_layout);
   if (err != hipSuccess) return err;
   hipLaunchKernelGGL(k_pool_finish, dim3((unsigned)((n_entries + 63) / 64 + 1)), dim3(kFinishThreads), 0, stream,
                      (const double *)partials, blocks, nr, nc, slots, n_slots, proposed, out_device);
diff --git a/metropolisengine_amd/csrc/me_internal.h b/metropolisengine_amd/csrc/me_internal.h
--- a/metropolisengine_amd/csrc/me_internal.h
+++ b/metropolisengine_amd/csrc/me_internal.h
@@ -4,6 +4,7 @@
 #include <stdint.h>
 
 #include "../../include/metropolis_engine.h"
+#include "me_state_layout.h"
 
 namespace me {
 
@@ -95,7 +96,7 @@
   bool has_user_reject;
   bool streams_packed;
   hipError_t (*cycle)(const StepLaunch &, const MeasureLaunch &, hipStream_t);
-  bool tiled_state;
+  int state_layout;
 };
 
 void register_kernel_set(const KernelSet *set);
@@ -105,17 +106,17 @@
 hipError_t launch_broadcast_rows(void *dst, const void *row_values, int rows, long long n, int dtype,
                                  hipStream_t stream);
 hipError_t launch_broadcast_tiled(void *dst, const void *entry_values, int entries, long long n, int dtype,
-                                  hipStream_t stream);
+                                  hipStream_t stream, int tile_chains = 64);
 hipError_t launch_pool_reduce(const void *x, long long n, int n_real, int n_complex, int dtype,
                               const unsigned long long *slots, long long n_slots, double proposed, double *partials,
                               double *out_device, hipStream_t stream,
                               hipError_t (*stage1)(const void *, long long, double *, int, hipStream_t) = nullptr,
-                              bool tiled_state = false);
+                              int state_layout = STATE_COMPONENT_MAJOR);
 int pool_reduce_blocks(long long n, int n_real, int n_complex);
 bool pool_reduce_supported(int n_real, int n_complex, int dtype);
 hipError_t launch_trace(const void *x, const void *energy, const void *width, long long n, int d, int n_terms,
                         int width_rows, int dtype, long long n_traced, long long stride, double *out, hipStream_t stream,
-                        bool tiled_state = false);
+                        int state_layout = STATE_COMPONENT_MAJOR);
 hipError_t launch_detect_equilibration(const double *series, long long n_series, long long length, int fast, int nskip,
                                        double *scratch, long long *t0_out, double *g_out, double *neff_out,
                                        hipStream_t stream);
diff --git a/metropolisengine_amd/csrc/me_kernels.hip b/metropolisengine_amd/csrc/me_kernels.hip
--- a/metropolisengine_amd/csrc/me_kernels.hip
+++ b/metropolisengine_amd/csrc/me_kernels.hip
@@ -152,18 +152,18 @@
       constexpr long long state_bytes = (long long)sizeof(R) * (D + 2);
       if constexpr (!INJECT && GROUP == GROUP_ALL) {
         if (state_bytes * l.n > 2 * cache_budget_bytes()) {
-          hipLaunchKernelGGL((k_step<R, NR, NC, Energy, CK_IDENTITY, INJECT, GROUP, true>), grid, block, 0, stream, a, en);
+          hipLaunchKernelGGL((k_step<R, NR, NC, Energy, CK_IDENTITY, INJECT, GROUP, true>), grid, block, (record_store_lds_bytes<R, D>(block.x)), stream, a, en);
           break;
         }
       }
-      hipLaunchKernelGGL((k_step<R, NR, NC, Energy, CK_IDENTITY, INJECT, GROUP>), grid, block, 0, stream, a, en);
+      hipLaunchKernelGGL((k_step<R, NR, NC, Energy, CK_IDENTITY, INJECT, GROUP>), grid, block, (record_store_lds_bytes<R, D>(block.x)), stream, a, en);
       break;
     }
-    case CK_SHARED: hipLaunchKernelGGL((k_step<R, NR, NC, Energy, CK_SHARED, INJECT, GROUP>), grid, block, 0, stream, a, en); break;
+    case CK_SHARED: hipLaunchKernelGGL((k_step<R, NR, NC, Energy, CK_SHARED, INJECT, GROUP>), grid, block, (record_store_lds_bytes<R, D>(block.x)), stream, a, en); break;
 #if ME_PER_CHAIN == 2
     case CK_PER_CHAIN: {
       if constexpr (INJECT) return hipErrorInvalidValue;
-      else hipLaunchKernelGGL((k_step<R, NR, NC, Energy, CK_PER_CHAIN_NT, INJECT, GROUP>), grid, block, 0, stream, a, en);
+      else hipLaunchKernelGGL((k_step<R, NR, NC, Energy, CK_PER_CHAIN_NT, INJECT, GROUP>), grid, block, (record_store_lds_bytes<R, D>(block.x)), stream, a, en);
       break;
     }
 #elif ME_PER_CHAIN
@@ -171,11 +171,11 @@
       constexpr long long per_chain_bytes = (long long)sizeof(R) * (D + 2 + NR * (NR + 1) / 2 + NC * NC);
       if constexpr (!INJECT) {
         if (per_chain_bytes * l.n > cache_budget_bytes()) {
-          hipLaunchKernelGGL((k_step<R, NR, NC, Energy, CK_PER_CHAIN_NT, INJECT, GROUP>), grid, block, 0, stream, a, en);
+          hipLaunchKernelGGL((k_step<R, NR, NC, Energy, CK_PER_CHAIN_NT, INJECT, GROUP>), grid, block, (record_store_lds_bytes<R, D>(block.x)), stream, a, en);
           break;
         }
       }
-      hipLaunchKernelGGL((k_step<R, NR, NC, Energy, CK_PER_CHAIN, INJECT, GROUP>), grid, block, 0, stream, a, en);
+      hipLaunchKernelGGL((k_step<R, NR, NC, Energy, CK_PER_CHAIN, INJECT, GROUP>), grid, block, (record_store_lds_bytes<R, D>(block.x)), stream, a, en);
       break;
     }
 #endif
@@ -396,9 +396,9 @@
       const dim3 grid(grid_for(l.n, l.grid_blocks, threads)), block(threads);
       auto launch = [&](auto ck) {
         constexpr int CK = decltype(ck)::value;
-        if (ntm) hipLaunchKernelGGL((k_cycle<R, NR, NC, Energy, CK, true, true>), grid, block, 0, stream, a, ma, en);
-        else if (nt) hipLaunchKernelGGL((k_cycle<R, NR, NC, Energy, CK, true, false>), grid, block, 0, stream, a, ma, en);
-        else hipLaunchKernelGGL((k_cycle<R, NR, NC, Energy, CK, false, false>), grid, block, 0, stream, a, ma, en);
+        if (ntm) hipLaunchKernelGGL((k_cycle<R, NR, NC, Energy, CK, true, true>), grid, block, (record_store_lds_bytes<R, D>(block.x)), stream, a, ma, en);
+        else if (nt) hipLaunchKernelGGL((k_cycle<R, NR, NC, Energy, CK, true, false>), grid, block, (record_store_lds_bytes<R, D>(block.x)), stream, a, ma, en);
+        else hipLaunchKernelGGL((k_cycle<R, NR, NC, Energy, CK, false, false>), grid, block, (record_store_lds_bytes<R, D>(block.x)), stream, a, ma, en);
       };
       if (l.cov_kind == CK_PER_CHAIN) launch(std::integral_constant<int, CK_PER_CHAIN>{});
       else launch(std::integral_constant<int, CK_IDENTITY>{});
@@ -503,12 +503,12 @@
 #if ME_ONLY_DTYPE != 64
 const KernelSet kSetF32 = {ME_SET_NAME, ME_F32, NR, NC, ME_PER_CHAIN != 0, (ME_PER_CHAIN != 0 || ME_TRACK_COV != 0), has_energy, energy_terms, step<float>,
                            (NC > 0 && ME_PER_CHAIN == 1) ? magphase<float> : nullptr, measure<float>, init_energy<float>,
-                           ME_PREPARE_MATRIX_F32, kHasUserReject, ME_PER_CHAIN == 2, cycle<float>, D >= kTiledStateDof};
+                           ME_PREPARE_MATRIX_F32, kHasUserReject, ME_PER_CHAIN == 2, cycle<float>, state_layout_of<float, D>()};
 #endif
 #if ME_ONLY_DTYPE != 32
 const KernelSet kSetF64 = {ME_SET_NAME, ME_F64, NR, NC, ME_PER_CHAIN != 0, (ME_PER_CHAIN != 0 || ME_TRACK_COV != 0), has_energy, energy_terms, step<double>,
                            (NC > 0 && ME_PER_CHAIN == 1) ? magphase<double> : nullptr, measure<double>, init_energy<double>,
-                           ME_PREPARE_MATRIX_F64, kHasUserReject, ME_PER_CHAIN == 2, cycle<double>, D >= kTiledStateDof};
+                           ME_PREPARE_MATRIX_F64, kHasUserReject, ME_PER_CHAIN == 2, cycle<double>, state_layout_of<double, D>()};
 #endif
 
 struct Registrar {
diff --git a/metropolisengine_amd/csrc/me_magphase.h b/metropolisengine_amd/csrc/me_magphase.h
--- a/metropolisengine_amd/csrc/me_magphase.h
+++ b/metropolisengine_amd/csrc/me_magphase.h
@@ -48,8 +48,7 @@
     const unsigned int coff = (unsigned int)c * (unsigned int)sizeof(R);
     const unsigned int xoff = fx.offset(c);
     R x[D], kdiag[NC];
-#pragma unroll
-    for (int d = 0; d < D; ++d) x[d] = fx.load(d, xoff);
+    fx.load_all(x, xoff);
 #pragma unroll
     for (int j = 0; j < NC; ++j) kdiag[j] = fcov.load(cdiag(PR, j), tiled_offset<R>(c, P));
     Ledger ledger;
diff --git a/metropolisengine_amd/csrc/me_state_layout.h b/metropolisengine_amd/csrc/me_state_layout.h
--- /dev/null
+++ b/metropolisengine_amd/csrc/me_state_layout.h
@@ -0,0 +1,36 @@
+#pragma once
+
+#include <stddef.h>
+#include <stdint.h>
+
+#if defined(__HIPCC__)
+#define ME_HOST_DEVICE __host__ __device__
+#else
+#define ME_HOST_DEVICE
+#endif
+
+namespace me {
+
+enum StateLayout { STATE_COMPONENT_MAJOR = 0, STATE_TILE_MAJOR = 1, STATE_CHAIN_MAJOR = 2 };
+
+ME_HOST_DEVICE inline long long state_offset(int layout, long long c, int row, int d, long long n) {
+  if (layout == STATE_TILE_MAJOR) return ((c >> 6) * (long long)d + row) * 64 + (c & 63);
+  if (layout == STATE_CHAIN_MAJOR) return c * (long long)d + row;
+  return (long long)row * n + c;
+}
+inline int state_tile_chains(int layout) { return layout == STATE_CHAIN_MAJOR ? 1 : 64; }
+
+struct TileSpan {
+  int64_t first_tile, n_tiles;
+  bool whole;
+};
+inline TileSpan tile_span(int64_t chain_begin, int64_t n_chains, int tile_chains, int64_t n) {
+  const int64_t T = tile_chains, end = chain_begin + n_chains;
+  return {chain_begin / T, (end - 1) / T - chain_begin / T + 1, chain_begin % T == 0 && (end % T == 0 || end == n)};
+}
+inline size_t tiled_index(int64_t c, int k, int entries, int tile_chains, int64_t first_tile) {
+  const int64_t T = tile_chains;
+  return (size_t)((c / T - first_tile) * entries * T + (int64_t)k * T + c % T);
+}
+
+}
```

Result: slower. 18.37 billion, median of 6 (-6.5%).
